# lzyhha/VisualCloze

Hardware: AMD Instinct MI355X
Metric: denoising-steps/sec (higher is better)
Workload: dtype bf16; 1 GPU; 384-grid-2x3 in-context, 30 solver points = 29 Flux evaluations per grid, L=512+3456 tokens, FLUX.1-Fill-dev geometry + LoRA r256 (merged), random-init weights, 1 independent grid(s) per GPU (data-parallel, no in-step collective); global_batch=1, seq_len=3968, parallelism=dp1

## Files before the change

visualcloze_amd/csrc/api.hip:

```cpp
#include "vcloze_internal.h"
#include <string.h>

static thread_local char g_err[512] = "";
#define ERRBUF g_err, (int)sizeof(g_err)
static inline hipStream_t S(void* s) { return (hipStream_t)s; }
static int hip_fail(const char* what, hipError_t e) {
  snprintf(g_err, sizeof(g_err), "%s: %s", what, hipGetErrorString(e));
  return VC_ERR_HIP;
}

extern "C" {

int vc_abi_version(void) { return VC_ABI_VERSION; }
const char* vc_last_error(void) { return g_err; }
void vc_struct_sizes(int32_t out[7]) {
  out[0] = (int32_t)sizeof(VcGemmProblem); out[1] = (int32_t)sizeof(VcGemmArgs); out[2] = (int32_t)sizeof(VcLnStream);
  out[3] = (int32_t)sizeof(VcAttention); out[4] = (int32_t)sizeof(VcFluxConfig); out[5] = (int32_t)sizeof(VcFluxInputs);
  out[6] = (int32_t)sizeof(VcFluxLaunchClass);
}

int vc_device_count(void) {
  int n = 0;
  hipError_t e = hipGetDeviceCount(&n);
  if (e != hipSuccess) { hip_fail("hipGetDeviceCount", e); return 0; }
  return n;
}
int vc_device_info(int dev, char* name, int namelen, int* cu_count, int64_t* hbm_bytes) {
  hipDeviceProp_t p;
  hipError_t e = hipGetDeviceProperties(&p, dev);
  if (e != hipSuccess) return hip_fail("hipGetDeviceProperties", e);
  if (name && namelen > 0) { strncpy(name, p.gcnArchName, namelen - 1); name[namelen - 1] = 0; }
  if (cu_count) *cu_count = p.multiProcessorCount;
  if (hbm_bytes) *hbm_bytes = (int64_t)p.totalGlobalMem;
  return VC_OK;
}

int vc_gemm(const VcGemmArgs* args, int tile_cfg, void* stream) {
  if (!args) { snprintf(g_err, sizeof(g_err), "gemm: null args"); return VC_ERR_ARG; }
  return vc_gemm_launch(*args, tile_cfg, S(stream), ERRBUF);
}
int vc_gemm_plan(const VcGemmArgs* args, int tile_cfg, int32_t out[8]) {
  if (!args || !out) { snprintf(g_err, sizeof(g_err), "gemm_plan: null argument"); return VC_ERR_ARG; }
  return vc_gemm_plan_impl(*args, tile_cfg, out, ERRBUF);
}
int vc_ln_modulate(const void* x, int64_t ldx, void* y, int64_t ldy, const void* shift, const void* scale,
                   int64_t mod_bstride, int32_t rows, int32_t D, int32_t rows_per_batch, const int32_t* step_ptr,
                   int64_t mod_step_stride, void* stream) {
  return vc_ln_modulate_launch(x, ldx, y, ldy, shift, scale, mod_bstride, rows, D, rows_per_batch, step_ptr,
                               mod_step_stride, S(stream), ERRBUF);
}
int vc_ln_modulate2(const VcLnStream* a, const VcLnStream* b, int64_t mod_bstride, int32_t D, const int32_t* step_ptr,
                    int64_t mod_step_stride, void* stream) {
  return vc_ln_modulate2_launch(a, b, mod_bstride, D, step_ptr, mod_step_stride, S(stream), ERRBUF);
}
int vc_qknorm_rope_vt(void* qkv, int64_t ld, int64_t bstride, const void* q_scale, const void* k_scale,
                      const void* q_scale2, const void* k_scale2, int32_t split, const float* rope,
                      int64_t rope_bstride, void* vt, int32_t B, int32_t L, int32_t Lpad, int32_t H, int32_t parts, void* stream) {
  return vc_qknorm_rope_vt_launch(qkv, ld, bstride, q_scale, k_scale, q_scale2, k_scale2, split, rope, rope_bstride, vt, B, L, Lpad, H,
                                  parts, S(stream), ERRBUF);
}
int vc_attention(const VcAttention* a, void* stream) {
  if (!a) { snprintf(g_err, sizeof(g_err), "attention: null args"); return VC_ERR_ARG; }
  return vc_attention_launch(*a, S(stream), ERRBUF);
}
int64_t vc_attention_scratch_bytes(void) { return vc_attention_scratch_bytes_impl(); }
int vc_timestep_embedding(const float* t, const float* freqs, void* out_bf16, int32_t n, int32_t half,
                          int32_t round_t_bf16, void* stream) {
  return vc_temb_launch(t, freqs, out_bf16, n, half, round_t_bf16, S(stream), ERRBUF);
}
int vc_silu(const void* x, void* y, int64_t n, void* stream) { return vc_silu_launch(x, y, n, S(stream), ERRBUF); }
int vc_act2d(const void* x, int64_t ldx, void* y, int64_t ldy, int32_t rows, int32_t cols, int32_t act, void* stream) {
  return vc_act2d_launch(x, ldx, y, ldy, rows, cols, act, S(stream), ERRBUF);
}
int vc_gate_residual(const void* y, int64_t ldy, const void* res, int64_t ldres, const void* gate, void* out, int64_t ldo,
                     int32_t rows, int32_t cols, const int32_t* step_ptr, int64_t gate_step_stride, void* stream) {
  return vc_gate_residual_launch(y, ldy, res, ldres, gate, out, ldo, rows, cols, step_ptr, gate_step_stride, S(stream), ERRBUF);
}
int vc_add3(const void* a, const void* b, const void* c, void* y, int64_t n, int64_t bn, int64_t cn, void* stream) {
  return vc_add3_launch(a, b, c, y, n, bn, cn, S(stream), ERRBUF);
}
int vc_copy(void* dst, const void* src, int64_t bytes, void* stream) {
  if (!dst || !src || bytes <= 0) { snprintf(g_err, sizeof(g_err), "copy: bad args"); return VC_ERR_ARG; }
  hipError_t e = hipMemcpyAsync(dst, src, (size_t)bytes, hipMemcpyDeviceToDevice, S(stream));
  return e == hipSuccess ? VC_OK : hip_fail("hipMemcpyAsync", e);
}
int vc_concat_cols(const void* x, int32_t cx, const void* cond, int32_t cc, void* out, int64_t rows, void* stream) {
  return vc_concat_cols_launch(x, cx, cond, cc, out, rows, S(stream), ERRBUF);
}
int vc_euler_step(void* x, const void* v, const float* dts, const int32_t* step_ptr, int64_t n, void* stream) {
  return vc_euler_launch(x, v, dts, step_ptr, n, S(stream), ERRBUF);
}
int vc_euler_step_f32(float* x32, void* shadow, const void* v, const float* dts, const int32_t* step_ptr, int64_t n, void* stream) {
  return vc_euler_f32_launch(x32, shadow, v, dts, step_ptr, n, S(stream), ERRBUF);
}
int vc_solver_evals(int method) {
  if (vc_evals_of(method)) return vc_evals_of(method);
  snprintf(g_err, sizeof(g_err), "solver_evals: unknown method %d (VC_SOLVER_EULER, VC_SOLVER_MIDPOINT, VC_SOLVER_RK4)", method);
  return VC_ERR_ARG;
}
int vc_ode_stage(int32_t method, int32_t stage, void* y, int32_t state_is_bf16, const void* v, void* k, void* y_in,
                 const float* dts, const int32_t* eval_ptr, int64_t n, void* stream) {
  return vc_ode_stage_launch(method, stage, y, state_is_bf16, v, k, y_in, dts, eval_ptr, n, S(stream), ERRBUF);
}
int vc_step_advance(int32_t* step_ptr, void* stream) { return vc_step_advance_launch(step_ptr, S(stream), ERRBUF); }
int vc_residual_change(const void* h0, const void* h1, const void* p, void* r, float* sums, float* metric, float* scratch, int32_t B,
                       int64_t n, void* stream) {
  return vc_residual_change_launch(h0, h1, p, r, sums, metric, scratch, B, n, S(stream), ERRBUF);
}
int vc_residual_sub(const void* a, int64_t a_bstride, const void* b, int64_t b_bstride, void* out, int64_t out_bstride, int32_t B,
                    int64_t n, void* stream) {
  return vc_residual_op_launch(0, a, a_bstride, b, b_bstride, out, out_bstride, B, n, S(stream), ERRBUF);
}
int vc_residual_add(const void* a, int64_t a_bstride, const void* b, int64_t b_bstride, void* out, int64_t out_bstride, int32_t B,
                    int64_t n, void* stream) {
  return vc_residual_op_launch(1, a, a_bstride, b, b_bstride, out, out_bstride, B, n, S(stream), ERRBUF);
}

int vc_sdedit_mix(const void* noise, const void* latent, float strength, void* out, int64_t n, void* stream) {
  return vc_sdedit_mix_launch(noise, latent, strength, out, n, S(stream), ERRBUF);
}
int vc_im2col3x3(const void* src, void* dst, int32_t H, int32_t W, int32_t C, int32_t up, void* stream) {
  return vc_im2col3x3_launch(src, dst, H, W, C, up, S(stream), ERRBUF);
}
int vc_groupnorm(const void* x, const void* gamma, const void* beta, void* y, void* scratch, int64_t scratch_bytes,
                 int64_t HW, int32_t C, int32_t G, float eps, int32_t swish, void* stream) {
  return vc_groupnorm_launch(x, gamma, beta, y, scratch, scratch_bytes, HW, C, G, eps, swish, S(stream), ERRBUF);
}
int vc_softmax_rows(void* x, int64_t ld, int32_t rows, int32_t cols, float scale, const void* bias, int64_t ld_bias,
                    int32_t causal_period, void* stream) {
  return vc_softmax_rows_launch(x, ld, rows, cols, scale, bias, ld_bias, causal_period, S(stream), ERRBUF);
}
int vc_embedding(const int32_t* ids, const void* table, int64_t ld_table, int32_t vocab, void* out, int32_t L, int32_t D, void* stream) {
  return vc_embedding_launch(ids, table, ld_table, vocab, out, L, D, S(stream), ERRBUF);
}
int vc_rmsnorm(const void* x, const void* weight, void* y, int32_t rows, int32_t D, float eps, void* stream) {
  return vc_rownorm_launch(x, weight, nullptr, y, rows, D, eps, 0, S(stream), ERRBUF);
}
int vc_layernorm(const void* x, const void* weight, const void* bias, void* y, int32_t rows, int32_t D, float eps, void* stream) {
  return vc_rownorm_launch(x, weight, bias, y, rows, D, eps, 1, S(stream), ERRBUF);
}
int vc_mul(const void* a, const void* b, void* y, int64_t n, void* stream) { return vc_ewise_launch(a, b, y, n, 0, S(stream), ERRBUF); }
int vc_add(const void* a, const void* b, void* y, int64_t n, void* stream) { return vc_ewise_launch(a, b, y, n, 1, S(stream), ERRBUF); }
int vc_quick_gelu(const void* x, void* y, int64_t n, void* stream) { return vc_ewise_launch(x, nullptr, y, n, 2, S(stream), ERRBUF); }
int vc_transpose(const void* src, int64_t ld_src, void* dst, int64_t ld_dst, int32_t rows, int32_t cols, void* stream) {
  return vc_transpose_launch(src, ld_src, dst, ld_dst, rows, cols, S(stream), ERRBUF);
}
int vc_nchw_to_nhwc(const void* src, int32_t src_is_f32, void* dst, int32_t C, int32_t Cp, int64_t HW, float div, float add, void* stream) {
  return vc_nchw_to_nhwc_launch(src, src_is_f32, dst, C, Cp, HW, div, add, S(stream), ERRBUF);
}
int vc_nhwc_to_nchw(const void* src, void* dst, int32_t dst_is_f32, int32_t C, int32_t Cp, int64_t HW, void* stream) {
  return vc_nhwc_to_nchw_launch(src, dst, dst_is_f32, C, Cp, HW, S(stream), ERRBUF);
}
int vc_gaussian_sample(const void* moments, int32_t Cp, const void* noise, void* out, int32_t Z, int64_t HW, float scale, float shift, void* stream) {
  return vc_gaussian_sample_launch(moments, Cp, noise, out, Z, HW, scale, shift, S(stream), ERRBUF);
}
int vc_conv3x3(const void* x, const void* w, const void* bias, void* out, int64_t ldc, const void* res, int64_t ldres,
               const void* gate, int32_t H, int32_t W, int32_t C, int32_t O, int32_t mode, void* stream) {
  return vc_conv3x3_launch(x, w, bias, out, ldc, res, ldres, gate, H, W, C, O, mode, S(stream), ERRBUF);
}
int vc_pack_latent(const void* latent, void* tokens, int32_t C, int32_t h, int32_t w, int64_t ld, int32_t col0, void* stream) {
  return vc_pack_latent_launch(latent, tokens, C, h, w, ld, col0, S(stream), ERRBUF);
}
int vc_pack_mask(const void* mask, void* tokens, int32_t H, int32_t W, int64_t ld, int32_t col0, void* stream) {
  return vc_pack_mask_launch(mask, tokens, H, W, ld, col0, S(stream), ERRBUF);
}
int vc_unpack_latent(const void* tokens, int64_t ld, int32_t col0, void* latent, int32_t C, int32_t h, int32_t w, void* stream) {
  return vc_unpack_latent_launch(tokens, ld, col0, latent, C, h, w, S(stream), ERRBUF);
}
int vc_lora_merge(const void* w, int32_t w_is_f32, int64_t ldw, const void* lora_a, int64_t lda, const void* lora_b, int64_t ldb,
                  float scale, void* out, int64_t ldo, const void* bias, int32_t bias_is_f32, const void* lora_b_bias, void* bias_out,
                  int32_t out_features, int32_t in_features, int32_t rank, void* stream) {
  return vc_lora_merge_launch(w, w_is_f32, ldw, lora_a, lda, lora_b, ldb, scale, out, ldo, bias, bias_is_f32, lora_b_bias, bias_out,
                              out_features, in_features, rank, S(stream), ERRBUF);
}

int vc_flux_create(const VcFluxConfig* cfg, void** handle) { return vc_flux_create_impl(cfg, handle, ERRBUF); }
int vc_flux_destroy(void* handle) { return vc_flux_destroy_impl(handle, ERRBUF); }
int vc_flux_bind_weight(void* handle, const char* name, const void* w, const void* bias, int32_t rows, int32_t cols, int64_t ldw) {
  return vc_flux_bind_weight_impl(handle, name, w, bias, rows, cols, ldw, ERRBUF);
}
int64_t vc_flux_mod_offset(void* handle, const char* module_name) { return vc_flux_mod_offset_impl(handle, module_name); }
int vc_flux_set_option(void* handle, const char* name, int32_t value) { return vc_flux_set_option_impl(handle, name, value, ERRBUF); }
int64_t vc_flux_workspace_bytes(void* handle, int32_t B, int32_t T, int32_t N, int32_t max_steps) {
  return vc_flux_workspace_bytes_impl(handle, B, T, N, max_steps);
}
int vc_flux_prepare(void* handle, const VcFluxInputs* in, void* workspace, int64_t workspace_bytes, void* stream) {
  return vc_flux_prepare_impl(handle, in, workspace, workspace_bytes, S(stream), ERRBUF);
}
int vc_flux_forward(void* handle, const void* img, const float* timesteps, int32_t timesteps_is_bf16, void* out, void* stream) {
  return vc_flux_forward_impl(handle, img, timesteps, timesteps_is_bf16, out, S(stream), ERRBUF);
}
int vc_flux_sample_begin(void* handle, const void* x, const void* cond, const float* t_grid, int32_t n_points, int32_t state_is_bf16,
                         void* stream) {
  return vc_flux_sample_begin_impl(handle, VC_SOLVER_EULER, x, cond, t_grid, n_points, state_is_bf16, S(stream), ERRBUF);
}
int vc_flux_sample_begin_ode(void* handle, int32_t method, const void* x, const void* cond, const float* t_grid, int32_t n_points,
                             int32_t state_is_bf16, void* stream) {
  return vc_flux_sample_begin_impl(handle, method, x, cond, t_grid, n_points, state_is_bf16, S(stream), ERRBUF);
}
int vc_flux_sample_steps(void* handle, int32_t n_steps, void* trajectory, void* stream) {
  return vc_flux_sample_steps_impl(handle, n_steps, trajectory, S(stream), ERRBUF);
}
int vc_flux_profile(void* handle, int32_t evaluations, VcFluxLaunchClass* out, int32_t capacity, int32_t* count, void* stream) {
  return vc_flux_profile_impl(handle, evaluations, out, capacity, count, S(stream), ERRBUF);
}
int vc_flux_sample_end(void* handle, void* x_out, void* stream) { return vc_flux_sample_end_impl(handle, x_out, S(stream), ERRBUF); }
int vc_flux_set_step_cache(void* handle, float threshold, int32_t max_consecutive) {
  return vc_flux_set_step_cache_impl(handle, threshold, max_consecutive, ERRBUF);
}
int vc_flux_step_cache_stats(void* handle, int32_t* computed, int32_t* reused, float* metrics, int32_t capacity) {
  return vc_flux_step_cache_stats_impl(handle, computed, reused, metrics, capacity, ERRBUF);
}
int vc_flux_sample_ode(void* handle, int32_t method, void* x, const void* cond, const float* t_grid, int32_t n_points,
                       int32_t state_is_bf16, void* trajectory, void* stream) {
  int rc = vc_flux_sample_begin_impl(handle, method, x, cond, t_grid, n_points, state_is_bf16, S(stream), ERRBUF);
  if (rc == VC_OK) rc = vc_flux_sample_steps_impl(handle, n_points - 1, trajectory, S(stream), ERRBUF);
  if (rc == VC_OK) rc = vc_flux_sample_end_impl(handle, x, S(stream), ERRBUF);
  return rc;
}
int vc_flux_sample_euler(void* handle, void* x, const void* cond, const float* t_grid, int32_t n_points, int32_t state_is_bf16,
                         void* trajectory, void* stream) {
  return vc_flux_sample_ode(handle, VC_SOLVER_EULER, x, cond, t_grid, n_points, state_is_bf16, trajectory, stream);
}

int vc_stream_create(void** stream) {
  if (!stream) { snprintf(g_err, sizeof(g_err), "stream_create: null"); return VC_ERR_ARG; }
  hipStream_t s;
  hipError_t e = hipStreamCreateWithFlags(&s, hipStreamNonBlocking);
  if (e != hipSuccess) return hip_fail("hipStreamCreate", e);
  *stream = (void*)s;
  return VC_OK;
}
int vc_stream_destroy(void* stream) {
  hipError_t e = hipStreamDestroy(S(stream));
  return e == hipSuccess ? VC_OK : hip_fail("hipStreamDestroy", e);
}
int vc_stream_sync(void* stream) {
  hipError_t e = hipStreamSynchronize(S(stream));
  return e == hipSuccess ? VC_OK : hip_fail("hipStreamSynchronize", e);
}
int vc_graph_begin(void* stream) {
  hipError_t e = hipStreamBeginCapture(S(stream), hipStreamCaptureModeThreadLocal);
  return e == hipSuccess ? VC_OK : hip_fail("hipStreamBeginCapture", e);
}
int vc_graph_end(void* stream, void** graph_exec) {
  if (!graph_exec) { snprintf(g_err, sizeof(g_err), "graph_end: null"); return VC_ERR_ARG; }
  hipGraph_t g = nullptr;
  hipError_t e = hipStreamEndCapture(S(stream), &g);
  if (e != hipSuccess) return hip_fail("hipStreamEndCapture", e);
  hipGraphExec_t ge = nullptr;
  e = hipGraphInstantiate(&ge, g, nullptr, nullptr, 0);
  (void)hipGraphDestroy(g);
  if (e != hipSuccess) return hip_fail("hipGraphInstantiate", e);
  *graph_exec = (void*)ge;
  return VC_OK;
}
int vc_graph_launch(void* graph_exec, void* stream) {
  hipError_t e = hipGraphLaunch((hipGraphExec_t)graph_exec, S(stream));
  return e == hipSuccess ? VC_OK : hip_fail("hipGraphLaunch", e);
}
int vc_graph_destroy(void* graph_exec) {
  hipError_t e = hipGraphExecDestroy((hipGraphExec_t)graph_exec);
  return e == hipSuccess ? VC_OK : hip_fail("hipGraphExecDestroy", e);
}
int vc_event_create(void** ev) {
  if (!ev) { snprintf(g_err, sizeof(g_err), "event_create: null"); return VC_ERR_ARG; }
  hipEvent_t e_;
  hipError_t e = hipEventCreate(&e_);
  if (e != hipSuccess) return hip_fail("hipEventCreate", e);
  *ev = (void*)e_;
  return VC_OK;
}
int vc_event_record(void* ev, void* stream) {
  hipError_t e = hipEventRecord((hipEvent_t)ev, S(stream));
  return e == hipSuccess ? VC_OK : hip_fail("hipEventRecord", e);
}
int vc_event_elapsed_ms(void* ev_start, void* ev_stop, float* ms) {
  hipError_t e = hipEventSynchronize((hipEvent_t)ev_stop);
  if (e != hipSuccess) return hip_fail("hipEventSynchronize", e);
  e = hipEventElapsedTime(ms, (hipEvent_t)ev_start, (hipEvent_t)ev_stop);
  return e == hipSuccess ? VC_OK : hip_fail("hipEventElapsedTime", e);
}
int vc_event_destroy(void* ev) {
  hipError_t e = hipEventDestroy((hipEvent_t)ev);
  return e == hipSuccess ? VC_OK : hip_fail("hipEventDestroy", e);
}

}
```

visualcloze_amd/csrc/flux_engine.hip:

```cpp
#include "common.h"
#include "vcloze_internal.h"
#include <math.h>
#include <string.h>
#include <string>
#include <unordered_map>
#include <vector>

namespace {

struct Lin {
  const void* w = nullptr;
  const void* b = nullptr;
  int N = 0, K = 0;
  int64_t ldw = 0;
};

struct DoubleW { Lin qkv[2], proj[2], mlp0[2], mlp2[2]; const void* qs[2]; const void* ks[2]; int64_t mod[2]; float bound; };
struct SingleW { Lin qkv, mlp, lin2; const void* qs; const void* ks; int64_t mod; float bound; };

struct Err {
  char* buf; int len;
};

struct Buffers {
  bf16_t *XI, *XT, *X, *XH, *QKV, *VT, *CAT, *HID, *TXT0, *XIN, *V, *XS, *COND, *MOD, *TEMB, *H1, *TVEC, *GVEC, *YVEC, *VEC, *GE, *GH, *YH, *KS, *YIN;
  float *ROPE, *TS, *DTS, *G32, *FREQS, *XS32;
  int32_t *STEP, *KVLEN, *KVGAP;
  bf16_t *SC_P = nullptr, *SC_R = nullptr, *SC_RS = nullptr;
  float *SC_PART = nullptr, *SC_METRIC = nullptr;
  void* ATT_SCRATCH = nullptr;
  int64_t att_scratch_bytes = 0;
  void* SK_WS = nullptr;
  int64_t sk_ws_bytes = 0;
};

struct Flux : Buffers {
  VcFluxConfig cfg{};
  int D = 0, H = 0, mlp = 0;
  int64_t n_mod = 0;
  std::unordered_map<std::string, Lin> bound;
  std::unordered_map<std::string, int64_t> mod_off;
  bool resolved = false;
  Lin img_in, txt_in, time_in[2], vector_in[2], guidance_in[2], final_lin, modulation;
  std::vector<DoubleW> dbl;
  std::vector<SingleW> sgl;
  int64_t final_mod = 0;
  int attn_variant = -1, tile_cfg = 0, fuse_qnorm = 2, fuse_vt = 1, qkv_heads = 0, fuse_knorm = 0, logit_bound_milli = 0, mlp_first = 0, splitk = 1, n_cu = 256;
  bool prepared = false;
  bool ws_sized = false;
  int B = 0, T = 0, N = 0, L = 0, Lp = 0, S = 0;
  bool ragged = false, gapped = false;
  char* base = nullptr;
  hipGraphExec_t graph = nullptr;
  struct Step { hipGraphExec_t g[3] = {nullptr, nullptr, nullptr}; } step;
  struct Key {
    char* base; int B, T, N, S, ragged, gapped, variant, tile, fuse, fuse_vt, state_f32, qkv_heads, fuse_knorm, bound, mlp_first, splitk, method, cache; hipStream_t s;
    bool operator==(const Key& o) const {
      return base == o.base && B == o.B && T == o.T && N == o.N && S == o.S && ragged == o.ragged && gapped == o.gapped &&
             variant == o.variant && tile == o.tile && fuse == o.fuse && fuse_vt == o.fuse_vt && state_f32 == o.state_f32 &&
             qkv_heads == o.qkv_heads && fuse_knorm == o.fuse_knorm && bound == o.bound && mlp_first == o.mlp_first && splitk == o.splitk && method == o.method && cache == o.cache && s == o.s;
    }
  } key{};
  std::vector<std::pair<Key, Step>> graphs;
  int steps_total = 0, steps_done = 0;
  bool state_f32 = false;
  int method = VC_SOLVER_EULER, evals = 1;
  float sc_threshold = 0.0f; int sc_max = 0;
  bool sc_on() const { return sc_threshold > 0.0f && sc_max != 0; }
  bool ws_cache = false;
  bool sc_active = false, sc_have = false;
  float sc_thr = 0.0f; int sc_lim = 0, sc_run = 0;
  int sc_computed = 0, sc_reused = 0;
  std::vector<float> sc_metrics;
  float* sc_host = nullptr;
  char* pinned = nullptr;
  size_t pinned_bytes = 0, pinned_used = 0;
  hipEvent_t staged = nullptr;
  bool staged_pending = false;
  struct ProfRec { int kind, epi, n, k; double flops, bytes; size_t e0; };
  bool prof_on = false;
  std::vector<hipEvent_t> prof_ev;
  size_t prof_used = 0;
  std::vector<ProfRec> prof_recs;
};

#define FAIL(code, ...)                         \
  do {                                          \
    snprintf(e.buf, e.len, __VA_ARGS__);        \
    return code;                                \
  } while (0)
#define TRY(x)                \
  do {                        \
    int rc_ = (x);            \
    if (rc_ != VC_OK) return rc_; \
  } while (0)
#define HIP(x, what)                                                        \
  do {                                                                      \
    hipError_t he_ = (x);                                                   \
    if (he_ != hipSuccess) FAIL(VC_ERR_HIP, what ": %s", hipGetErrorString(he_)); \
  } while (0)

inline int64_t align256(int64_t v) { return (v + 255) & ~(int64_t)255; }

struct Carver {
  char* base; int64_t off = 0;
  template <class T> T* take(int64_t count) {
    T* p = base ? (T*)(base + off) : nullptr;
    off += align256(count * (int64_t)sizeof(T));
    return p;
  }
};

int64_t carve(Buffers& f, const Flux& g, char* base, int B, int T, int N, int S) {
  const int64_t D = g.D, H = g.H, mlp = g.mlp, L = T + N, Lp = (L + 63) / 64 * 64;
  const int64_t in_ch = g.cfg.in_channels, out_ch = g.cfg.out_channels;
  Carver c{base};
  f.XI = c.take<bf16_t>(B * N * D);          f.XT = c.take<bf16_t>(B * T * D);
  f.X = c.take<bf16_t>(B * L * D);           f.XH = c.take<bf16_t>(B * L * D);
  f.QKV = c.take<bf16_t>(B * L * 3 * D);     f.VT = c.take<bf16_t>(B * H * 128 * Lp);
  f.CAT = c.take<bf16_t>(B * L * (D + mlp)); f.HID = c.take<bf16_t>(B * L * mlp);
  f.TXT0 = c.take<bf16_t>(B * T * D);        f.XIN = c.take<bf16_t>(B * N * in_ch);
  f.V = c.take<bf16_t>(B * N * out_ch);      f.XS = c.take<bf16_t>(B * N * out_ch);
  f.COND = c.take<bf16_t>(B * N * (in_ch - out_ch));
  f.MOD = c.take<bf16_t>((int64_t)S * B * g.n_mod);
  f.TEMB = c.take<bf16_t>((int64_t)S * B * 256);
  f.H1 = c.take<bf16_t>((int64_t)S * B * D); f.TVEC = c.take<bf16_t>((int64_t)S * B * D);
  f.VEC = c.take<bf16_t>((int64_t)S * B * D);
  f.GVEC = c.take<bf16_t>(B * D);            f.YVEC = c.take<bf16_t>(B * D);
  f.GE = c.take<bf16_t>(B * 256);            f.GH = c.take<bf16_t>(B * D);  f.YH = c.take<bf16_t>(B * D);
  f.ROPE = c.take<float>(B * L * 128);
  f.TS = c.take<float>((int64_t)S * B);      f.DTS = c.take<float>(S);
  f.G32 = c.take<float>(B);                  f.FREQS = c.take<float>(128);
  f.XS32 = c.take<float>(B * N * out_ch);
  f.KS = c.take<bf16_t>(3 * B * N * out_ch); f.YIN = c.take<bf16_t>(B * N * out_ch);
  f.STEP = c.take<int32_t>(1);               f.KVLEN = c.take<int32_t>(B);  f.KVGAP = c.take<int32_t>(2 * B);
  f.att_scratch_bytes = vc_attention_scratch_bytes_impl();
  f.ATT_SCRATCH = c.take<char>(f.att_scratch_bytes);
  auto sk = g.bound.find("splitk_ws");
  if (sk != g.bound.end()) { f.SK_WS = const_cast<void*>(sk->second.w); f.sk_ws_bytes = (int64_t)sk->second.N * sk->second.K * 4; }
  else { f.SK_WS = c.take<char>(VC_GEMM_SPLITK_WS_BYTES); f.sk_ws_bytes = VC_GEMM_SPLITK_WS_BYTES; }
  if (g.sc_on()) {
    f.SC_P = c.take<bf16_t>(B * N * D); f.SC_R = c.take<bf16_t>(B * N * D); f.SC_RS = c.take<bf16_t>(B * N * D);
    f.SC_PART = c.take<float>((int64_t)B * 2 * VC_RESIDUAL_CHANGE_MAX_BLOCKS); f.SC_METRIC = c.take<float>(1);
  }
  return c.off;
}

int find(Flux& f, const std::string& name, Lin& out, int N, int K, bool need_bias, Err e) {
  auto it = f.bound.find(name);
  if (it == f.bound.end()) FAIL(VC_ERR_STATE, "flux: weight '%s' is not bound", name.c_str());
  out = it->second;
  if (out.N != N || out.K != K) FAIL(VC_ERR_ARG, "flux: weight '%s' is [%d, %d], expected [%d, %d]", name.c_str(), out.N, out.K, N, K);
  if (need_bias && !out.b) FAIL(VC_ERR_ARG, "flux: weight '%s' needs a bias", name.c_str());
  return VC_OK;
}
int find_scale(Flux& f, const std::string& name, const void*& out, Err e) {
  auto it = f.bound.find(name);
  if (it == f.bound.end()) FAIL(VC_ERR_STATE, "flux: scale '%s' is not bound", name.c_str());
  if (it->second.N * it->second.K != 128) FAIL(VC_ERR_ARG, "flux: scale '%s' must hold 128 values", name.c_str());
  out = it->second.w;
  return VC_OK;
}

void layout_modulation(Flux& f) {
  int64_t o = 0;
  for (int i = 0; i < f.cfg.depth; ++i) {
    f.mod_off["double_blocks." + std::to_string(i) + ".img_mod.lin"] = o; o += 6 * f.D;
    f.mod_off["double_blocks." + std::to_string(i) + ".txt_mod.lin"] = o; o += 6 * f.D;
  }
  for (int i = 0; i < f.cfg.depth_single_blocks; ++i) { f.mod_off["single_blocks." + std::to_string(i) + ".modulation.lin"] = o; o += 3 * f.D; }
  f.mod_off["final_layer.adaLN_modulation.1"] = o; o += 2 * f.D;
  f.n_mod = o;
}

int scale_absmax(const void* dev, double& out, Err e) {
  uint16_t h[128];
  HIP(hipMemcpy(h, dev, sizeof(h), hipMemcpyDeviceToHost), "hipMemcpy (QK-norm scale)");
  out = 0;
  bool nan = false;
  for (int i = 0; i < 128; ++i) {
    uint32_t u = (uint32_t)h[i] << 16;
    float v;
    memcpy(&v, &u, 4);
    const double a = v < 0 ? -(double)v : (double)v;
    if (a != a) nan = true;
    else if (a > out) out = a;
  }
  if (nan) out = 1e30;
  return VC_OK;
}
inline float logit_bound_of(double qmax, double kmax) { return (float)(1.02 * 11.313708498984761 * 1.4426950408889634 * qmax * kmax); }

int resolve(Flux& f, Err e) {
  if (f.resolved) return VC_OK;
  const int D = f.D, mlp = f.mlp;
  TRY(find(f, "img_in", f.img_in, D, f.cfg.in_channels, false, e));
  TRY(find(f, "txt_in", f.txt_in, D, f.cfg.context_in_dim, false, e));
  TRY(find(f, "time_in.in_layer", f.time_in[0], D, 256, false, e));
  TRY(find(f, "time_in.out_layer", f.time_in[1], D, D, false, e));
  TRY(find(f, "vector_in.in_layer", f.vector_in[0], D, f.cfg.vec_in_dim, false, e));
  TRY(find(f, "vector_in.out_layer", f.vector_in[1], D, D, false, e));
  if (f.cfg.guidance_embed) {
    TRY(find(f, "guidance_in.in_layer", f.guidance_in[0], D, 256, false, e));
    TRY(find(f, "guidance_in.out_layer", f.guidance_in[1], D, D, false, e));
  }
  TRY(find(f, "final_layer.linear", f.final_lin, f.cfg.out_channels, D, false, e));
  TRY(find(f, "modulation", f.modulation, (int)f.n_mod, D, false, e));
  f.dbl.assign(f.cfg.depth, DoubleW{});
  for (int i = 0; i < f.cfg.depth; ++i) {
    const std::string pf = "double_blocks." + std::to_string(i) + ".";
    const char* st[2] = {"img", "txt"};
    for (int k = 0; k < 2; ++k) {
      const std::string a = pf + st[k] + "_attn.", m = pf + st[k] + "_mlp.";
      TRY(find(f, a + "qkv", f.dbl[i].qkv[k], 3 * D, D, false, e));
      TRY(find(f, a + "proj", f.dbl[i].proj[k], D, D, false, e));
      TRY(find(f, m + "0", f.dbl[i].mlp0[k], mlp, D, false, e));
      TRY(find(f, m + "2", f.dbl[i].mlp2[k], D, mlp, false, e));
      TRY(find_scale(f, a + "norm.query_norm.scale", f.dbl[i].qs[k], e));
      TRY(find_scale(f, a + "norm.key_norm.scale", f.dbl[i].ks[k], e));
      f.dbl[i].mod[k] = f.mod_off[pf + st[k] + "_mod.lin"];
    }
    double q[2], k2[2];
    for (int k = 0; k < 2; ++k) { TRY(scale_absmax(f.dbl[i].qs[k], q[k], e)); TRY(scale_absmax(f.dbl[i].ks[k], k2[k], e)); }
    f.dbl[i].bound = logit_bound_of(q[0] > q[1] ? q[0] : q[1], k2[0] > k2[1] ? k2[0] : k2[1]);
  }
  f.sgl.assign(f.cfg.depth_single_blocks, SingleW{});
  for (int i = 0; i < f.cfg.depth_single_blocks; ++i) {
    const std::string pf = "single_blocks." + std::to_string(i) + ".";
    Lin l1;
    TRY(find(f, pf + "linear1", l1, 3 * D + mlp, D, false, e));
    SingleW& w = f.sgl[i];
    w.qkv = l1; w.qkv.N = 3 * D;
    w.mlp = l1; w.mlp.N = mlp;
    w.mlp.w = (const bf16_t*)l1.w + (int64_t)3 * D * l1.ldw;
    w.mlp.b = l1.b ? (const void*)((const bf16_t*)l1.b + 3 * D) : nullptr;
    TRY(find(f, pf + "linear2", w.lin2, D, D + mlp, false, e));
    TRY(find_scale(f, pf + "norm.query_norm.scale", w.qs, e));
    TRY(find_scale(f, pf + "norm.key_norm.scale", w.ks, e));
    w.mod = f.mod_off[pf + "modulation.lin"];
    double q, k;
    TRY(scale_absmax(w.qs, q, e)); TRY(scale_absmax(w.ks, k, e));
    w.bound = logit_bound_of(q, k);
  }
  f.final_mod = f.mod_off["final_layer.adaLN_modulation.1"];
  f.resolved = true;
  return VC_OK;
}

int attention_variant(const Flux& f);
bool kn_in_gemm(const Flux& f) { return f.fuse_knorm && f.qkv_heads > 0 && (attention_variant(f) & 8); }
bool qn_in_gemm(const Flux& f) { return kn_in_gemm(f) && f.fuse_qnorm >= 2; }
int qkv_epi(const Flux& f) { return f.fuse_vt || f.qkv_heads > 0 ? VC_EPI_QKV : VC_EPI_BIAS; }
void with_vt(Flux& f, VcGemmProblem& p, int rows, int row0, const void* q_scale, const void* k_scale) {
  if (f.fuse_vt) { p.vt = f.VT; p.vt_bstride = (int64_t)f.H * 128 * f.Lp; p.vt_col0 = 2 * f.D; p.vt_lpad = f.Lp; }
  if (f.qkv_heads > 0) {
    p.kn_heads = f.qkv_heads;
    if (kn_in_gemm(f)) { p.kn_scale = k_scale; p.kn_rope = f.ROPE; p.kn_rope_bstride = (int64_t)f.L * 128; }
    if (qn_in_gemm(f)) { p.qn_scale = q_scale; p.qn_prescale = 1; }
  }
  if (f.fuse_vt || f.qkv_heads > 0) { p.vt_rpb = rows; p.vt_row0 = row0; }
}

VcGemmProblem prob(const void* A, int64_t lda, const Lin& w, void* C, int64_t ldc, int M) {
  VcGemmProblem p;
  memset(&p, 0, sizeof(p));
  p.A = A; p.W = w.w; p.bias = w.b; p.C = C;
  p.lda = lda; p.ldw = w.ldw; p.ldc = ldc;
  p.M = M; p.N = w.N; p.K = w.K;
  p.rows_per_batch = M;
  return p;
}
int prof_event(Flux& f, hipStream_t s, Err e) {
  if (f.prof_used == f.prof_ev.size()) {
    hipEvent_t ev;
    HIP(hipEventCreate(&ev), "hipEventCreate");
    f.prof_ev.push_back(ev);
  }
  HIP(hipEventRecord(f.prof_ev[f.prof_used++], s), "hipEventRecord");
  return VC_OK;
}
int prof_open(Flux& f, hipStream_t s, int kind, int epi, int n, int k, double flops, double bytes, Err e) {
  if (!f.prof_on) return VC_OK;
  f.prof_recs.push_back(Flux::ProfRec{kind, epi, n, k, flops, bytes, f.prof_used});
  return prof_event(f, s, e);
}
int prof_close(Flux& f, hipStream_t s, Err e) { return f.prof_on ? prof_event(f, s, e) : VC_OK; }

int gemm(Flux& f, const VcGemmProblem* ps, int n, int epi, const int32_t* step_ptr, int64_t gate_step_stride, hipStream_t s, Err e) {
  VcGemmArgs a;
  memset(&a, 0, sizeof(a));
  for (int i = 0; i < n; ++i) a.p[i] = ps[i];
  a.nprob = n; a.epi = epi; a.step_ptr = step_ptr; a.gate_step_stride = gate_step_stride;
  if (f.splitk) { a.splitk_ws = f.SK_WS; a.splitk_ws_bytes = f.sk_ws_bytes; }
  double flops = 0;
  for (int i = 0; i < n; ++i) flops += 2.0 * ps[i].M * ps[i].N * ps[i].K;
  TRY(prof_open(f, s, VC_LAUNCH_GEMM, epi, ps[0].N, ps[0].K, flops, 0, e));
  TRY(vc_gemm_launch(a, f.tile_cfg, s, e.buf, e.len));
  return prof_close(f, s, e);
}
int lin(Flux& f, const Lin& w, const void* A, int64_t lda, void* C, int64_t ldc, int M, int epi, hipStream_t s, Err e) {
  VcGemmProblem p = prob(A, lda, w, C, ldc, M);
  return gemm(f, &p, 1, epi, nullptr, 0, s, e);
}

struct Ctx {
  const int32_t* step_ptr;
  hipStream_t s;
  int64_t mss;
};
inline const bf16_t* modp(Flux& f, int64_t off, int idx) { return f.MOD + off + (int64_t)idx * f.D; }

int ln2(Flux& f, const Ctx& c, const DoubleW& w, int idx, Err e) {
  VcLnStream a{f.XI, f.D, f.XH, f.D, modp(f, w.mod[0], idx), modp(f, w.mod[0], idx + 1), f.B * f.N, f.N};
  VcLnStream b{f.XT, f.D, f.XH + (int64_t)f.B * f.N * f.D, f.D, modp(f, w.mod[1], idx), modp(f, w.mod[1], idx + 1), f.B * f.T, f.T};
  TRY(prof_open(f, c.s, VC_LAUNCH_LN_MODULATE, 0, 0, 0, 0, 4.0 * f.B * f.L * f.D, e));
  TRY(vc_ln_modulate2_launch(&a, &b, f.n_mod, f.D, c.step_ptr, c.mss, c.s, e.buf, e.len));
  return prof_close(f, c.s, e);
}
int ln1(Flux& f, const Ctx& c, int64_t mod, Err e) {
  TRY(prof_open(f, c.s, VC_LAUNCH_LN_MODULATE, 0, 0, 0, 0, 4.0 * f.B * f.L * f.D, e));
  TRY(vc_ln_modulate_launch(f.X, f.D, f.XH, f.D, modp(f, mod, 0), modp(f, mod, 1), f.n_mod, f.B * f.L, f.D, f.L, c.step_ptr, c.mss,
                            c.s, e.buf, e.len));
  return prof_close(f, c.s, e);
}

int attention_variant(const Flux& f) {
  if (f.attn_variant >= 0) return f.attn_variant;
  const int items = ((f.L + 255) / 256) * f.H * f.B;
  return items >= f.n_cu ? 28 : 2 * items >= f.n_cu ? 8 : 3;
}

int attention(Flux& f, const Ctx& c, const void* q1, const void* k1, const void* q2, const void* k2, int split, float block_bound, Err e) {
  const int variant = attention_variant(f);
  const bool fused_q = (variant & 8) && f.fuse_qnorm, q_done = qn_in_gemm(f);
  const int64_t ld = 3 * f.D, ldo = f.D + f.mlp;
  const int parts = (kn_in_gemm(f) ? 0 : VC_QKN_K) | (fused_q ? 0 : VC_QKN_Q) | (f.fuse_vt ? 0 : VC_QKN_VT);
  if (parts)
    TRY(vc_qknorm_rope_vt_launch(f.QKV, ld, f.L * ld, q1, k1, q2, k2, split, f.ROPE, (int64_t)f.L * 128, f.VT, f.B, f.L, f.Lp, f.H,
                                 parts, c.s, e.buf, e.len));
  VcAttention a;
  memset(&a, 0, sizeof(a));
  a.qkv = f.QKV; a.ld = ld; a.bstride = f.L * ld;
  a.vt = f.VT; a.out = f.CAT; a.ldo = ldo; a.out_bstride = f.L * ldo;
  a.kv_len = f.ragged ? f.KVLEN : nullptr;
  a.kv_gap = f.gapped ? f.KVGAP : nullptr;
  a.B = f.B; a.L = f.L; a.Lpad = f.Lp; a.H = f.H; a.variant = variant;
  a.scratch = f.ATT_SCRATCH; a.scratch_bytes = f.att_scratch_bytes;
  if (q_done) a.q_prescaled = 1;
  else if (fused_q) { a.q_scale = q1; a.q_scale2 = q2; a.split = split; a.rope = f.ROPE; a.rope_bstride = (int64_t)f.L * 128; }
  const float cap = (float)f.logit_bound_milli * 1e-3f;
  a.logit_bound = f.logit_bound_milli > 0 ? (block_bound < cap ? block_bound : cap) : 0.0f;
  if (f.logit_bound_milli > 0 && !(block_bound < 1e30f)) a.logit_bound = 1e30f;
  TRY(prof_open(f, c.s, VC_LAUNCH_ATTENTION, variant, 0, 0, 4.0 * f.L * f.L * f.D * f.B, 0, e));
  TRY(vc_attention_launch(a, c.s, e.buf, e.len));
  return prof_close(f, c.s, e);
}

int double_block(Flux& f, const Ctx& c, const DoubleW& w, Err e) {
  const int B = f.B, T = f.T, N = f.N, L = f.L, D = f.D, mlp = f.mlp;
  const int64_t ldq = 3 * D, ldc = D + mlp;
  bf16_t* XH_I = f.XH; bf16_t* XH_T = f.XH + (int64_t)B * N * D;
  bf16_t* HID_I = f.HID; bf16_t* HID_T = f.HID + (int64_t)B * N * mlp;
  bf16_t* streams[2] = {f.XI, f.XT};
  const int rows[2] = {N, T};
  TRY(ln2(f, c, w, 0, e));
  {
    VcGemmProblem p[2] = {prob(XH_I, D, w.qkv[0], f.QKV + (int64_t)T * ldq, ldq, B * N), prob(XH_T, D, w.qkv[1], f.QKV, ldq, B * T)};
    p[0].c_rpb = N; p[1].c_rpb = T;
    p[0].c_bstride = p[1].c_bstride = (int64_t)L * ldq;
    with_vt(f, p[0], N, T, w.qs[0], w.ks[0]); with_vt(f, p[1], T, 0, w.qs[1], w.ks[1]);
    TRY(gemm(f, p, 2, qkv_epi(f), nullptr, 0, c.s, e));
  }
  TRY(attention(f, c, w.qs[1], w.ks[1], w.qs[0], w.ks[0], T, w.bound, e));
  {
    VcGemmProblem p[2] = {prob(f.CAT + (int64_t)T * ldc, ldc, w.proj[0], f.XI, D, B * N), prob(f.CAT, ldc, w.proj[1], f.XT, D, B * T)};
    for (int k = 0; k < 2; ++k) {
      p[k].res = streams[k]; p[k].ldres = D; p[k].gate = modp(f, w.mod[k], 2); p[k].gate_bstride = f.n_mod;
      p[k].rows_per_batch = rows[k]; p[k].a_rpb = rows[k]; p[k].a_bstride = (int64_t)L * ldc;
    }
    TRY(gemm(f, p, 2, VC_EPI_GATE_RES, c.step_ptr, c.mss, c.s, e));
  }
  TRY(ln2(f, c, w, 3, e));
  {
    VcGemmProblem p[2] = {prob(XH_I, D, w.mlp0[0], HID_I, mlp, B * N), prob(XH_T, D, w.mlp0[1], HID_T, mlp, B * T)};
    TRY(gemm(f, p, 2, VC_EPI_GELU, nullptr, 0, c.s, e));
  }
  {
    VcGemmProblem p[2] = {prob(HID_I, mlp, w.mlp2[0], f.XI, D, B * N), prob(HID_T, mlp, w.mlp2[1], f.XT, D, B * T)};
    for (int k = 0; k < 2; ++k) {
      p[k].res = streams[k]; p[k].ldres = D; p[k].gate = modp(f, w.mod[k], 5); p[k].gate_bstride = f.n_mod; p[k].rows_per_batch = rows[k];
    }
    TRY(gemm(f, p, 2, VC_EPI_GATE_RES, c.step_ptr, c.mss, c.s, e));
  }
  return VC_OK;
}

int single_block(Flux& f, const Ctx& c, const SingleW& w, Err e) {
  const int M = f.B * f.L, D = f.D, mlp = f.mlp;
  const int64_t ldc = D + mlp;
  TRY(ln1(f, c, w.mod, e));
  {
    VcGemmProblem p = prob(f.XH, D, w.qkv, f.QKV, 3 * D, M);
    with_vt(f, p, f.L, 0, w.qs, w.ks);
    TRY(gemm(f, &p, 1, qkv_epi(f), nullptr, 0, c.s, e));
  }
  if (f.mlp_first) TRY(lin(f, w.mlp, f.XH, D, f.CAT + D, ldc, M, VC_EPI_GELU, c.s, e));
  TRY(attention(f, c, w.qs, w.ks, nullptr, nullptr, 0, w.bound, e));
  if (!f.mlp_first) TRY(lin(f, w.mlp, f.XH, D, f.CAT + D, ldc, M, VC_EPI_GELU, c.s, e));
  VcGemmProblem p = prob(f.CAT, ldc, w.lin2, f.X, D, M);
  p.res = f.X; p.ldres = D; p.gate = modp(f, w.mod, 2); p.gate_bstride = f.n_mod; p.rows_per_batch = f.L;
  return gemm(f, &p, 1, VC_EPI_GATE_RES, c.step_ptr, c.mss, c.s, e);
}

int d2d(void* dst, const void* src, int64_t bytes, hipStream_t s, Err e) {
  HIP(hipMemcpyAsync(dst, src, (size_t)bytes, hipMemcpyDeviceToDevice, s), "hipMemcpyAsync");
  return VC_OK;
}

int eval_inputs(Flux& f, bool concat, const void* img_rows, hipStream_t s, Err e) {
  const int B = f.B, T = f.T, N = f.N, D = f.D;
  const int in_ch = f.cfg.in_channels, out_ch = f.cfg.out_channels;
  if (concat) TRY(vc_concat_cols_launch(f.method == VC_SOLVER_EULER ? f.XS : f.YIN, out_ch, f.COND, in_ch - out_ch, f.XIN, (int64_t)B * N, s, e.buf, e.len));
  TRY(d2d(f.XT, f.TXT0, (int64_t)B * T * D * 2, s, e));
  return lin(f, f.img_in, img_rows ? img_rows : f.XIN, in_ch, f.XI, D, B * N, VC_EPI_BIAS, s, e);
}
int eval_blocks(Flux& f, const Ctx& c, size_t first, Err e) {
  const int B = f.B, T = f.T, N = f.N, L = f.L, D = f.D;
  hipStream_t s = c.s;
  for (size_t i = first; i < f.dbl.size(); ++i) TRY(double_block(f, c, f.dbl[i], e));
  for (int b = 0; b < B; ++b) {
    TRY(d2d(f.X + (int64_t)b * L * D, f.XT + (int64_t)b * T * D, (int64_t)T * D * 2, s, e));
    TRY(d2d(f.X + ((int64_t)b * L + T) * D, f.XI + (int64_t)b * N * D, (int64_t)N * D * 2, s, e));
  }
  for (auto& w : f.sgl) TRY(single_block(f, c, w, e));
  return VC_OK;
}
int eval_output(Flux& f, const Ctx& c, void* out, bool euler, Err e) {
  const int B = f.B, T = f.T, N = f.N, L = f.L, D = f.D;
  const int out_ch = f.cfg.out_channels;
  const int32_t* step_ptr = c.step_ptr;
  hipStream_t s = c.s;
  TRY(ln1(f, c, f.final_mod, e));
  VcGemmProblem p = prob(f.XH + (int64_t)T * D, D, f.final_lin, out ? out : f.V, out_ch, B * N);
  p.a_rpb = N; p.a_bstride = (int64_t)L * D;
  TRY(gemm(f, &p, 1, VC_EPI_BIAS, nullptr, 0, s, e));
  if (euler && f.method != VC_SOLVER_EULER) {
    TRY(vc_ode_stage_launch(f.method, -1, f.state_f32 ? (void*)f.XS32 : (void*)f.XS, !f.state_f32, f.V, f.KS, f.YIN, f.DTS, step_ptr,
                            (int64_t)B * N * out_ch, s, e.buf, e.len));
    TRY(vc_step_advance_launch((int32_t*)step_ptr, s, e.buf, e.len));
  } else if (euler) {
    if (f.state_f32) TRY(vc_euler_f32_launch(f.XS32, f.XS, f.V, f.DTS, step_ptr, (int64_t)B * N * out_ch, s, e.buf, e.len));
    else TRY(vc_euler_launch(f.XS, f.V, f.DTS, step_ptr, (int64_t)B * N * out_ch, s, e.buf, e.len));
    TRY(vc_step_advance_launch((int32_t*)step_ptr, s, e.buf, e.len));
  }
  return VC_OK;
}
int evaluate(Flux& f, const int32_t* step_ptr, bool concat, const void* img_rows, void* out, bool euler, hipStream_t s, Err e) {
  Ctx c{step_ptr, s, (int64_t)f.B * f.n_mod};
  TRY(eval_inputs(f, concat, img_rows, s, e));
  TRY(eval_blocks(f, c, 0, e));
  return eval_output(f, c, out, euler, e);
}

int cache_head(Flux& f, hipStream_t s, Err e) {
  const int64_t nd = (int64_t)f.N * f.D;
  Ctx c{f.STEP, s, (int64_t)f.B * f.n_mod};
  TRY(eval_inputs(f, true, nullptr, s, e));
  TRY(d2d(f.X, f.XI, f.B * nd * 2, s, e));
  TRY(double_block(f, c, f.dbl[0], e));
  TRY(vc_residual_change_launch(f.X, f.XI, f.SC_P, f.SC_RS, nullptr, f.SC_METRIC, f.SC_PART, f.B, nd, s, e.buf, e.len));
  HIP(hipMemcpyAsync(f.sc_host, f.SC_METRIC, sizeof(float), hipMemcpyDeviceToHost, s), "hipMemcpyAsync(D2H)");
  return VC_OK;
}
int cache_tail_compute(Flux& f, bool euler, hipStream_t s, Err e) {
  const int64_t nd = (int64_t)f.N * f.D;
  Ctx c{f.STEP, s, (int64_t)f.B * f.n_mod};
  TRY(d2d(f.SC_P, f.SC_RS, f.B * nd * 2, s, e));
  TRY(d2d(f.SC_RS, f.XI, f.B * nd * 2, s, e));
  TRY(eval_blocks(f, c, 1, e));
  TRY(vc_residual_op_launch(0, f.X + (int64_t)f.T * f.D, (int64_t)f.L * f.D, f.SC_RS, nd, f.SC_R, nd, f.B, nd, s, e.buf, e.len));
  return eval_output(f, c, nullptr, euler, e);
}
int cache_tail_reuse(Flux& f, bool euler, hipStream_t s, Err e) {
  const int64_t nd = (int64_t)f.N * f.D;
  Ctx c{f.STEP, s, (int64_t)f.B * f.n_mod};
  TRY(vc_residual_op_launch(1, f.XI, nd, f.SC_R, nd, f.X + (int64_t)f.T * f.D, (int64_t)f.L * f.D, f.B, nd, s, e.buf, e.len));
  return eval_output(f, c, nullptr, euler, e);
}

int stage_begin(Flux& f, size_t bytes, Err e) {
  if (f.staged_pending) { HIP(hipEventSynchronize(f.staged), "hipEventSynchronize"); f.staged_pending = false; }
  if (bytes > f.pinned_bytes) {
    if (f.pinned) (void)hipHostFree(f.pinned);
    f.pinned = nullptr; f.pinned_bytes = 0;
    HIP(hipHostMalloc((void**)&f.pinned, bytes, hipHostMallocDefault), "hipHostMalloc");
    f.pinned_bytes = bytes;
  }
  f.pinned_used = 0;
  return VC_OK;
}
template <class T> T* stage_take(Flux& f, size_t count) {
  T* p = (T*)(f.pinned + f.pinned_used);
  f.pinned_used += (size_t)align256((int64_t)(count * sizeof(T)));
  return p;
}
int stage_send(Flux& f, void* dst, const void* staged, size_t bytes, hipStream_t s, Err e) {
  HIP(hipMemcpyAsync(dst, staged, bytes, hipMemcpyHostToDevice, s), "hipMemcpyAsync(H2D)");
  return VC_OK;
}
int stage_end(Flux& f, hipStream_t s, Err e) {
  HIP(hipEventRecord(f.staged, s), "hipEventRecord");
  f.staged_pending = true;
  return VC_OK;
}

inline float bf16_round(float v) {
  uint32_t u;
  memcpy(&u, &v, 4);
  u += 0x7fffu + ((u >> 16) & 1u);
  u &= 0xffff0000u;
  memcpy(&v, &u, 4);
  return v;
}

int time_precompute(Flux& f, int S, int timesteps_is_bf16, hipStream_t s, Err e) {
  const int B = f.B, D = f.D, M = S * B;
  TRY(vc_temb_launch(f.TS, f.FREQS, f.TEMB, M, 128, timesteps_is_bf16, s, e.buf, e.len));
  TRY(lin(f, f.time_in[0], f.TEMB, 256, f.H1, D, M, VC_EPI_SILU, s, e));
  TRY(lin(f, f.time_in[1], f.H1, D, f.TVEC, D, M, VC_EPI_BIAS, s, e));
  if (f.cfg.guidance_embed)
    TRY(vc_add3_launch(f.TVEC, f.GVEC, f.YVEC, f.VEC, (int64_t)M * D, (int64_t)B * D, (int64_t)B * D, s, e.buf, e.len));
  else
    TRY(vc_add3_launch(f.TVEC, f.YVEC, nullptr, f.VEC, (int64_t)M * D, (int64_t)B * D, 1, s, e.buf, e.len));
  TRY(vc_silu_launch(f.VEC, f.H1, (int64_t)M * D, s, e.buf, e.len));
  return lin(f, f.modulation, f.H1, D, f.MOD, f.n_mod, M, VC_EPI_BIAS, s, e);
}

constexpr size_t MAX_GRAPHS = 4;
void drop_prof(Flux& f) {
  for (auto ev : f.prof_ev) (void)hipEventDestroy(ev);
  f.prof_ev.clear();
}
void drop_graph(Flux& f) {
  for (auto& g : f.graphs)
    for (auto ge : g.second.g) if (ge) (void)hipGraphExecDestroy(ge);
  f.graphs.clear();
  f.graph = nullptr;
  f.step = Flux::Step{};
}

template <class F> int capture(hipStream_t s, hipGraphExec_t& out, Err e, F issue) {
  HIP(hipStreamBeginCapture(s, hipStreamCaptureModeThreadLocal), "hipStreamBeginCapture");
  const int rc = issue();
  hipGraph_t g = nullptr;
  hipError_t he = hipStreamEndCapture(s, &g);
  if (rc != VC_OK) { if (g) (void)hipGraphDestroy(g); return rc; }
  HIP(he, "hipStreamEndCapture");
  he = hipGraphInstantiate(&out, g, nullptr, nullptr, 0);
  (void)hipGraphDestroy(g);
  HIP(he, "hipGraphInstantiate");
  return VC_OK;
}
int step_graph(Flux& f, hipStream_t s, Err e) {
  Flux::Key k{f.base, f.B, f.T, f.N, f.S, f.ragged, f.gapped, attention_variant(f), f.tile_cfg, f.fuse_qnorm, f.fuse_vt, f.state_f32,
              f.qkv_heads, f.fuse_knorm, f.logit_bound_milli, f.mlp_first, f.splitk, f.method, f.sc_active, s};
  for (size_t i = 0; i < f.graphs.size(); ++i)
    if (f.graphs[i].first == k) {
      auto hit = f.graphs[i];
      f.graphs.erase(f.graphs.begin() + i);
      f.graphs.insert(f.graphs.begin(), hit);
      f.step = hit.second; f.graph = f.step.g[0]; f.key = k;
      return VC_OK;
    }
  f.graph = nullptr;
  f.step = Flux::Step{};
  Flux::Step st;
  int rc = VC_OK;
  if (!f.sc_active) {
    TRY(evaluate(f, f.STEP, true, nullptr, nullptr, false, s, e));
    rc = capture(s, st.g[0], e, [&] { return evaluate(f, f.STEP, true, nullptr, nullptr, true, s, e); });
  } else {
    TRY(cache_head(f, s, e));
    TRY(cache_tail_compute(f, false, s, e));
    TRY(cache_tail_reuse(f, false, s, e));
    rc = capture(s, st.g[0], e, [&] { return cache_head(f, s, e); });
    if (rc == VC_OK) rc = capture(s, st.g[1], e, [&] { return cache_tail_compute(f, true, s, e); });
    if (rc == VC_OK) rc = capture(s, st.g[2], e, [&] { return cache_tail_reuse(f, true, s, e); });
  }
  if (rc != VC_OK) {
    for (auto ge : st.g) if (ge) (void)hipGraphExecDestroy(ge);
    return rc;
  }
  if (f.graphs.size() >= MAX_GRAPHS) {
    for (auto ge : f.graphs.back().second.g) if (ge) (void)hipGraphExecDestroy(ge);
    f.graphs.pop_back();
  }
  f.graphs.insert(f.graphs.begin(), {k, st});
  f.step = st; f.graph = st.g[0]; f.key = k;
  return VC_OK;
}

}

#define H(handle)                                                         \
  Err e{err, errlen};                                                     \
  if (!(handle)) FAIL(VC_ERR_ARG, "flux: null handle");                   \
  Flux& f = *(Flux*)(handle)

int vc_flux_create_impl(const VcFluxConfig* cfg, void** handle, char* err, int errlen) {
  Err e{err, errlen};
  if (!cfg || !handle) FAIL(VC_ERR_ARG, "flux_create: null argument");
  if (cfg->hidden_size <= 0 || cfg->num_heads <= 0 || cfg->hidden_size != cfg->num_heads * 128)
    FAIL(VC_ERR_ARG, "flux_create: hidden_size must be num_heads * 128 (the gfx950 attention kernels are specialised for head_dim 128)");
  if (cfg->axes_dim[0] + cfg->axes_dim[1] + cfg->axes_dim[2] != 128 || (cfg->axes_dim[0] | cfg->axes_dim[1] | cfg->axes_dim[2]) & 1)
    FAIL(VC_ERR_ARG, "flux_create: axes_dim must be even and sum to 128");
  if (cfg->in_channels <= cfg->out_channels || cfg->out_channels <= 0 || cfg->depth < 0 || cfg->depth_single_blocks < 0 || cfg->mlp_hidden <= 0)
    FAIL(VC_ERR_ARG, "flux_create: bad channel / depth configuration");
  Flux* f = new Flux();
  f->cfg = *cfg;
  f->D = cfg->hidden_size; f->H = cfg->num_heads; f->mlp = cfg->mlp_hidden;
  layout_modulation(*f);
  int dev = 0;
  hipDeviceProp_t p;
  if (hipGetDevice(&dev) != hipSuccess || hipGetDeviceProperties(&p, dev) != hipSuccess) {
    delete f;
    FAIL(VC_ERR_HIP, "flux_create: no ROCm device");
  }
  f->n_cu = p.multiProcessorCount;
  if (hipEventCreateWithFlags(&f->staged, hipEventDisableTiming) != hipSuccess) { delete f; FAIL(VC_ERR_HIP, "flux_create: hipEventCreate failed"); }
  *handle = f;
  return VC_OK;
}

int vc_flux_destroy_impl(void* handle, char* err, int errlen) {
  H(handle);
  if (f.staged_pending) (void)hipEventSynchronize(f.staged);
  drop_graph(f);
  drop_prof(f);
  if (f.pinned) (void)hipHostFree(f.pinned);
  if (f.sc_host) (void)hipHostFree(f.sc_host);
  if (f.staged) (void)hipEventDestroy(f.staged);
  delete &f;
  return VC_OK;
}

int vc_flux_bind_weight_impl(void* handle, const char* name, const void* w, const void* bias, int32_t rows, int32_t cols, int64_t ldw,
                             char* err, int errlen) {
  H(handle);
  if (!name || !w || rows <= 0 || cols <= 0 || ldw < cols) FAIL(VC_ERR_ARG, "flux_bind_weight: bad arguments for '%s'", name ? name : "?");
  if (!strcmp(name, "splitk_ws") && f.ws_sized && f.bound.find("splitk_ws") == f.bound.end())
    FAIL(VC_ERR_STATE, "flux_bind_weight: bind 'splitk_ws' BEFORE the first vc_flux_workspace_bytes / vc_flux_prepare (it changes the size and "
                       "layout of every workspace)");
  Lin l;
  l.w = w; l.b = bias; l.N = rows; l.K = cols; l.ldw = ldw;
  f.bound[name] = l;
  f.resolved = false;
  f.prepared = false;
  drop_graph(f);
  return VC_OK;
}

int64_t vc_flux_mod_offset_impl(void* handle, const char* name) {
  if (!handle) return -1;
  Flux& f = *(Flux*)handle;
  if (!name) return f.n_mod;
  auto it = f.mod_off.find(name);
  return it == f.mod_off.end() ? -1 : it->second;
}

int vc_flux_set_option_impl(void* handle, const char* name, int32_t value, char* err, int errlen) {
  H(handle);
  if (!name) FAIL(VC_ERR_ARG, "flux_set_option: null name");
  if (!strcmp(name, "attn_variant")) f.attn_variant = value;
  else if (!strcmp(name, "tile_cfg")) f.tile_cfg = value;
  else if (!strcmp(name, "fuse_qnorm")) f.fuse_qnorm = value < 0 ? 0 : value > 2 ? 2 : value;
  else if (!strcmp(name, "fuse_vt")) f.fuse_vt = value != 0;
  else if (!strcmp(name, "qkv_heads")) {
    if (value != 0 && value != f.H) FAIL(VC_ERR_ARG, "flux_set_option: qkv_heads must be 0 or num_heads = %d", f.H);
    f.qkv_heads = value;
  } else if (!strcmp(name, "fuse_knorm")) f.fuse_knorm = value != 0;
  else if (!strcmp(name, "logit_bound_milli")) f.logit_bound_milli = value > 0 ? value : 0;
  else if (!strcmp(name, "mlp_first")) f.mlp_first = value != 0;
  else if (!strcmp(name, "splitk")) f.splitk = value != 0;
  else FAIL(VC_ERR_ARG, "flux_set_option: unknown option '%s'", name);
  return VC_OK;
}

int64_t vc_flux_workspace_bytes_impl(void* handle, int32_t B, int32_t T, int32_t N, int32_t max_steps) {
  if (!handle || B <= 0 || T <= 0 || N <= 0 || max_steps <= 0) return -1;
  Buffers tmp;
  ((Flux*)handle)->ws_sized = true;
  return carve(tmp, *(Flux*)handle, nullptr, B, T, N, max_steps);
}

int vc_flux_prepare_impl(void* handle, const VcFluxInputs* in, void* workspace, int64_t workspace_bytes, hipStream_t s, char* err, int errlen) {
  H(handle);
  if (!in || !workspace) FAIL(VC_ERR_ARG, "flux_prepare: null argument");
  f.ws_sized = true;
  const int B = in->B, T = in->T, N = in->N, S = in->max_steps;
  if (B <= 0 || T <= 0 || N <= 0 || S <= 0) FAIL(VC_ERR_ARG, "flux_prepare: B, T, N, max_steps must be positive");
  if (!in->txt || !in->y || !in->img_ids || !in->txt_ids) FAIL(VC_ERR_ARG, "flux_prepare: txt, y, img_ids, txt_ids are required");
  if (f.cfg.guidance_embed && !in->guidance) FAIL(VC_ERR_ARG, "Didn't get guidance strength for guidance distilled model.");
  if (in->kv_gap && !in->kv_len) FAIL(VC_ERR_ARG, "flux_prepare: kv_gap needs kv_len");
  if ((uintptr_t)workspace & 255) FAIL(VC_ERR_ARG, "flux_prepare: workspace must be 256-byte aligned");
  TRY(resolve(f, e));
  f.prepared = false;
  const int64_t need = carve(f, f, (char*)workspace, B, T, N, S);
  if (workspace_bytes < need) FAIL(VC_ERR_ARG, "flux_prepare: workspace of %lld bytes, %lld needed", (long long)workspace_bytes, (long long)need);
  f.base = (char*)workspace;
  f.ws_cache = f.sc_on();
  f.B = B; f.T = T; f.N = N; f.L = T + N; f.Lp = (f.L + 63) / 64 * 64; f.S = S;
  const int L = f.L, D = f.D;
  f.ragged = f.gapped = false;
  for (int b = 0; b < B; ++b) {
    const int kv = in->kv_len ? in->kv_len[b] : L;
    if (kv < 0 || kv > L) FAIL(VC_ERR_ARG, "flux_prepare: kv_len[%d] = %d outside [0, %d]", b, kv, L);
    if (kv < L) f.ragged = true;
    if (in->kv_gap) {
      const int lo = in->kv_gap[2 * b], hi = in->kv_gap[2 * b + 1];
      if (lo < 0 || lo > hi || hi > kv) FAIL(VC_ERR_ARG, "flux_prepare: kv_gap[%d] = (%d, %d) must lie inside [0, kv_len = %d)", b, lo, hi, kv);
      if (hi > lo) f.gapped = true;
    }
  }
  if (f.gapped) f.ragged = true;
  const size_t n_rope = (size_t)B * L * 128;
  TRY(stage_begin(f, (n_rope + 128 + 4 * B + 64) * sizeof(float) + 8 * 256, e));
  float* rope = stage_take<float>(f, n_rope);
  {
    int pair0 = 0;
    std::vector<float> table;
    std::vector<int> slot((size_t)B * L);
    for (int ax = 0; ax < 3; ++ax) {
      const int half = f.cfg.axes_dim[ax] / 2, d = f.cfg.axes_dim[ax];
      std::unordered_map<float, int> seen;
      std::vector<float> values;
      for (int b = 0; b < B; ++b)
        for (int r = 0; r < L; ++r) {
          const float id = r < T ? in->txt_ids[((size_t)b * T + r) * 3 + ax] : in->img_ids[((size_t)b * N + (r - T)) * 3 + ax];
          auto it = seen.find(id);
          if (it == seen.end()) { it = seen.emplace(id, (int)values.size()).first; values.push_back(id); }
          slot[(size_t)b * L + r] = it->second;
        }
      table.resize(values.size() * (size_t)half * 2);
      for (int j = 0; j < half; ++j) {
        const double omega = 1.0 / pow((double)f.cfg.theta, (double)(2 * j) / (double)d);
        for (size_t v = 0; v < values.size(); ++v) {
          const double ang = (double)values[v] * omega;
          table[(v * half + j) * 2] = (float)cos(ang);
          table[(v * half + j) * 2 + 1] = (float)sin(ang);
        }
      }
      for (size_t row = 0; row < (size_t)B * L; ++row)
        memcpy(rope + (row * 64 + pair0) * 2, table.data() + (size_t)slot[row] * half * 2, (size_t)half * 2 * sizeof(float));
      pair0 += half;
    }
  }
  float* freqs = stage_take<float>(f, 128);
  for (int k = 0; k < 128; ++k)
    freqs[k] = (float)exp((double)((float)(-log(10000.0)) * (float)k / 128.0f));
  int32_t* kvl = stage_take<int32_t>(f, B);
  int32_t* gap = stage_take<int32_t>(f, 2 * B);
  float* g32 = stage_take<float>(f, B);
  for (int b = 0; b < B; ++b) {
    kvl[b] = in->kv_len ? in->kv_len[b] : L;
    gap[2 * b] = in->kv_gap ? in->kv_gap[2 * b] : 0;
    gap[2 * b + 1] = in->kv_gap ? in->kv_gap[2 * b + 1] : 0;
    g32[b] = in->guidance ? in->guidance[b] : 0.0f;
  }
  TRY(stage_send(f, f.ROPE, rope, n_rope * sizeof(float), s, e));
  {
    auto it = f.bound.find("timestep_freqs");
    if (it != f.bound.end()) {
      if (it->second.N * it->second.K != 128) FAIL(VC_ERR_ARG, "flux_prepare: 'timestep_freqs' must hold 128 f32 values");
      TRY(d2d(f.FREQS, it->second.w, 128 * sizeof(float), s, e));
    } else {
      TRY(stage_send(f, f.FREQS, freqs, 128 * sizeof(float), s, e));
    }
  }
  TRY(stage_send(f, f.KVLEN, kvl, B * sizeof(int32_t), s, e));
  TRY(stage_send(f, f.KVGAP, gap, 2 * B * sizeof(int32_t), s, e));
  TRY(stage_send(f, f.G32, g32, B * sizeof(float), s, e));
  TRY(stage_end(f, s, e));
  HIP(hipMemsetAsync(f.VT, 0, (size_t)B * f.H * 128 * f.Lp * 2, s), "hipMemsetAsync");
  HIP(hipMemsetAsync((char*)f.ATT_SCRATCH + vc_attention_flags_offset_impl(), 0, (size_t)vc_attention64_flags_bytes_impl(f.n_cu), s), "hipMemsetAsync");
  TRY(lin(f, f.txt_in, in->txt, f.cfg.context_in_dim, f.TXT0, D, B * T, VC_EPI_BIAS, s, e));
  if (f.cfg.guidance_embed) {
    TRY(vc_temb_launch(f.G32, f.FREQS, f.GE, B, 128, in->guidance_is_bf16, s, e.buf, e.len));
    TRY(lin(f, f.guidance_in[0], f.GE, 256, f.GH, D, B, VC_EPI_SILU, s, e));
    TRY(lin(f, f.guidance_in[1], f.GH, D, f.GVEC, D, B, VC_EPI_BIAS, s, e));
  }
  TRY(lin(f, f.vector_in[0], in->y, f.cfg.vec_in_dim, f.YH, D, B, VC_EPI_SILU, s, e));
  TRY(lin(f, f.vector_in[1], f.YH, D, f.YVEC, D, B, VC_EPI_BIAS, s, e));
  f.prepared = true;
  f.steps_total = f.steps_done = 0;
  return VC_OK;
}

int vc_flux_forward_impl(void* handle, const void* img, const float* timesteps, int32_t timesteps_is_bf16, void* out, hipStream_t s,
                         char* err, int errlen) {
  H(handle);
  if (!f.prepared) FAIL(VC_ERR_STATE, "flux_forward: call vc_flux_prepare first");
  if (!img || !timesteps || !out) FAIL(VC_ERR_ARG, "flux_forward: null argument");
  TRY(stage_begin(f, f.B * sizeof(float) + 256, e));
  float* ts = stage_take<float>(f, f.B);
  for (int b = 0; b < f.B; ++b) ts[b] = timesteps[b];
  TRY(stage_send(f, f.TS, ts, f.B * sizeof(float), s, e));
  TRY(stage_end(f, s, e));
  TRY(time_precompute(f, 1, timesteps_is_bf16, s, e));
  f.steps_total = f.steps_done = 0;
  return evaluate(f, nullptr, false, img, out, false, s, e);
}

void stage_times(int method, float t0, float t1, float dt, float* out) {
#pragma clang fp contract(off)
  out[0] = t0;
  if (method == VC_SOLVER_MIDPOINT) {
    volatile float half_dt = 0.5f * dt;
    out[1] = t0 + half_dt;
  } else if (method == VC_SOLVER_RK4) {
    volatile float a = dt * (float)(1.0 / 3.0), b = dt * (float)(2.0 / 3.0);
    out[1] = t0 + a; out[2] = t0 + b; out[3] = t1;
  }
}

int vc_flux_sample_begin_impl(void* handle, int32_t method, const void* x, const void* cond, const float* t_grid, int32_t n_points,
                              int32_t state_is_bf16, hipStream_t s, char* err, int errlen) {
  H(handle);
  const int E = vc_evals_of(method);
  if (!E) FAIL(VC_ERR_ARG, "flux_sample: unknown solver method %d (VC_SOLVER_EULER, VC_SOLVER_MIDPOINT, VC_SOLVER_RK4)", method);
  if (!f.prepared) FAIL(VC_ERR_STATE, "flux_sample: call vc_flux_prepare first");
  if (!x || !cond || !t_grid) FAIL(VC_ERR_ARG, "flux_sample: null argument");
  const int S = n_points - 1, B = f.B;
  if (S < 1 || (int64_t)S * E > f.S)
    FAIL(VC_ERR_ARG, "flux_sample: %d steps of %d evaluation(s), the prepared workspace holds 1..%d evaluations", S, E, f.S);
  const bool cached = f.sc_on();
  if (cached && method != VC_SOLVER_EULER)
    FAIL(VC_ERR_ARG, "flux_sample: the step cache works with VC_SOLVER_EULER only (method %d): turn it off with vc_flux_set_step_cache(handle, 0, 0)", method);
  if (cached && f.dbl.empty()) FAIL(VC_ERR_ARG, "flux_sample: the step cache needs at least one double block");
  if (cached && !f.ws_cache)
    FAIL(VC_ERR_STATE, "flux_sample: the step cache was turned on after vc_flux_prepare: ask vc_flux_workspace_bytes and prepare again");
  if (cached && !f.sc_host) HIP(hipHostMalloc((void**)&f.sc_host, 256, hipHostMallocDefault), "hipHostMalloc");
  const int SE = S * E;
  TRY(stage_begin(f, ((size_t)SE * B + S) * sizeof(float) + 512, e));
  float* ts = stage_take<float>(f, (size_t)SE * B);
  float* dts = stage_take<float>(f, S);
  for (int i = 0; i < S; ++i) {
    dts[i] = t_grid[i + 1] - t_grid[i];
    float te[4];
    stage_times(method, t_grid[i], t_grid[i + 1], dts[i], te);
    for (int j = 0; j < E; ++j) {
      const float tm = 1.0f - (state_is_bf16 ? bf16_round(te[j]) : te[j]);
      for (int b = 0; b < B; ++b) ts[((size_t)i * E + j) * B + b] = tm;
    }
  }
  TRY(stage_send(f, f.TS, ts, (size_t)SE * B * sizeof(float), s, e));
  TRY(stage_send(f, f.DTS, dts, S * sizeof(float), s, e));
  TRY(stage_end(f, s, e));
  TRY(time_precompute(f, SE, 0, s, e));
  const int64_t n = (int64_t)B * f.N;
  f.state_f32 = !state_is_bf16;
  f.method = method; f.evals = E;
  if (f.state_f32) {
    TRY(d2d(f.XS32, x, n * f.cfg.out_channels * 4, s, e));
    TRY(vc_euler_f32_launch(f.XS32, f.XS, nullptr, nullptr, nullptr, n * f.cfg.out_channels, s, e.buf, e.len));
  } else {
    TRY(d2d(f.XS, x, n * f.cfg.out_channels * 2, s, e));
  }
  if (E > 1) TRY(d2d(f.YIN, f.XS, n * f.cfg.out_channels * 2, s, e));
  TRY(d2d(f.COND, cond, n * (f.cfg.in_channels - f.cfg.out_channels) * 2, s, e));
  HIP(hipMemsetAsync(f.STEP, 0, sizeof(int32_t), s), "hipMemsetAsync");
  f.sc_active = cached; f.sc_thr = f.sc_threshold; f.sc_lim = f.sc_max;
  f.sc_have = false; f.sc_run = f.sc_computed = f.sc_reused = 0;
  f.sc_metrics.clear();
  if (s) TRY(step_graph(f, s, e));
  if (cached) HIP(hipMemsetAsync(f.SC_P, 0, (size_t)n * f.D * 2, s), "hipMemsetAsync");
  f.steps_total = S; f.steps_done = 0;
  return VC_OK;
}

static int cached_step(Flux& f, hipStream_t s, Err e) {
  if (s) HIP(hipGraphLaunch(f.step.g[0], s), "hipGraphLaunch");
  else TRY(cache_head(f, s, e));
  HIP(hipStreamSynchronize(s), "hipStreamSynchronize");
  const float m = *(volatile float*)f.sc_host;
  const bool reuse = f.sc_have && m < f.sc_thr && (f.sc_lim < 0 || f.sc_run < f.sc_lim);
  f.sc_metrics.push_back(f.sc_have ? m : NAN);
  if (s) HIP(hipGraphLaunch(f.step.g[reuse ? 2 : 1], s), "hipGraphLaunch");
  else if (reuse) TRY(cache_tail_reuse(f, true, s, e));
  else TRY(cache_tail_compute(f, true, s, e));
  if (reuse) { ++f.sc_reused; ++f.sc_run; }
  else { ++f.sc_computed; f.sc_run = 0; f.sc_have = true; }
  return VC_OK;
}

int vc_flux_sample_steps_impl(void* handle, int32_t n_steps, void* trajectory, hipStream_t s, char* err, int errlen) {
  H(handle);
  if (!f.prepared || f.steps_total == 0) FAIL(VC_ERR_STATE, "flux_sample_steps: call vc_flux_sample_begin first");
  if (n_steps < 0 || f.steps_done + n_steps > f.steps_total)
    FAIL(VC_ERR_ARG, "flux_sample_steps: %d more steps after %d of %d", n_steps, f.steps_done, f.steps_total);
  if (s && (!f.graph || f.key.s != s)) FAIL(VC_ERR_STATE, "flux_sample_steps: the step was captured on another stream");
  const int64_t state_bytes = (int64_t)f.B * f.N * f.cfg.out_channels * (f.state_f32 ? 4 : 2);
  const void* state = f.state_f32 ? (const void*)f.XS32 : (const void*)f.XS;
  for (int i = 0; i < n_steps; ++i) {
    for (int j = 0; j < f.evals; ++j) {
      if (f.sc_active) { TRY(cached_step(f, s, e)); continue; }
      if (s) HIP(hipGraphLaunch(f.graph, s), "hipGraphLaunch");
      else TRY(evaluate(f, f.STEP, true, nullptr, nullptr, true, s, e));
      ++f.sc_computed;
    }
    if (trajectory) TRY(d2d((char*)trajectory + (int64_t)i * state_bytes, state, state_bytes, s, e));
    ++f.steps_done;
  }
  return VC_OK;
}

int vc_flux_sample_end_impl(void* handle, void* x_out, hipStream_t s, char* err, int errlen) {
  H(handle);
  if (!f.prepared || f.steps_total == 0) FAIL(VC_ERR_STATE, "flux_sample_end: no sample in flight");
  if (!x_out) FAIL(VC_ERR_ARG, "flux_sample_end: null output");
  if (f.state_f32) return d2d(x_out, f.XS32, (int64_t)f.B * f.N * f.cfg.out_channels * 4, s, e);
  return d2d(x_out, f.XS, (int64_t)f.B * f.N * f.cfg.out_channels * 2, s, e);
}

int vc_flux_set_step_cache_impl(void* handle, float threshold, int32_t max_consecutive, char* err, int errlen) {
  H(handle);
  if (threshold != threshold) FAIL(VC_ERR_ARG, "flux_set_step_cache: threshold is NaN");
  f.sc_threshold = threshold > 0.0f ? threshold : 0.0f;
  f.sc_max = max_consecutive;
  return VC_OK;
}

int vc_flux_step_cache_stats_impl(void* handle, int32_t* computed, int32_t* reused, float* metrics, int32_t capacity, char* err, int errlen) {
  H(handle);
  if (capacity < 0 || (capacity > 0 && !metrics)) FAIL(VC_ERR_ARG, "flux_step_cache_stats: bad arguments");
  if (computed) *computed = f.sc_computed;
  if (reused) *reused = f.sc_reused;
  const int done = f.sc_computed + f.sc_reused;
  for (int i = 0; i < capacity; ++i) metrics[i] = i < done && i < (int)f.sc_metrics.size() ? f.sc_metrics[i] : NAN;
  return VC_OK;
}

int vc_flux_profile_impl(void* handle, int32_t evaluations, VcFluxLaunchClass* out, int32_t capacity, int32_t* count, hipStream_t s,
                         char* err, int errlen) {
  H(handle);
  if (!f.prepared || f.steps_total == 0) FAIL(VC_ERR_STATE, "flux_profile: call vc_flux_sample_begin first");
  if (!out || !count || capacity <= 0 || evaluations <= 0) FAIL(VC_ERR_ARG, "flux_profile: bad argument");
  TRY(evaluate(f, f.STEP, true, nullptr, nullptr, false, s, e));
  f.prof_recs.clear();
  f.prof_used = 0;
  f.prof_on = true;
  int rc = VC_OK;
  for (int i = 0; i < evaluations && rc == VC_OK; ++i) rc = evaluate(f, f.STEP, true, nullptr, nullptr, false, s, e);
  f.prof_on = false;
  if (rc != VC_OK) return rc;
  HIP(hipStreamSynchronize(s), "hipStreamSynchronize");
  int n = 0;
  for (const auto& r : f.prof_recs) {
    float ms = 0.f;
    HIP(hipEventElapsedTime(&ms, f.prof_ev[r.e0], f.prof_ev[r.e0 + 1]), "hipEventElapsedTime");
    const float us = ms * 1e3f;
    int j = 0;
    while (j < n && !(out[j].kind == r.kind && out[j].epi == r.epi && out[j].n == r.n && out[j].k == r.k)) ++j;
    if (j == n) {
      if (n == capacity) FAIL(VC_ERR_ARG, "flux_profile: more than %d launch classes", capacity);
      memset(&out[n], 0, sizeof(out[n]));
      out[n].kind = r.kind; out[n].epi = r.epi; out[n].n = r.n; out[n].k = r.k;
      out[n].min_us = us; out[n].max_us = us;
      ++n;
    }
    out[j].launches += 1;
    out[j].flops += r.flops;
    out[j].bytes += r.bytes;
    out[j].total_us += us;
    if (us < out[j].min_us) out[j].min_us = us;
    if (us > out[j].max_us) out[j].max_us = us;
  }
  *count = n;
  return VC_OK;
}
```

visualcloze_amd/csrc/norm.hip:

```cpp
#include "common.h"
#include "vcloze_internal.h"

namespace {

struct LnStream2 {
  const bf16_t* x; long ldx; bf16_t* y; long ldy; const bf16_t* shift; const bf16_t* scale; int rows; int rows_per_batch;
};

template <int NCH>
__global__ __launch_bounds__(256) void ln_modulate_kernel(const bf16_t* __restrict__ x, long ldx, bf16_t* __restrict__ y,
                                                          long ldy, const bf16_t* __restrict__ shift,
                                                          const bf16_t* __restrict__ scale, long mod_bstride, int rows,
                                                          int D, int rows_per_batch, const int* __restrict__ step_ptr,
                                                          long mod_step_stride, const LnStream2 second) {
  const int lane = threadIdx.x & 63;
  int row = blockIdx.x * 4 + (threadIdx.x >> 6);
  if (row >= rows) {
    row -= rows;
    if (row >= second.rows) return;
    x = second.x; ldx = second.ldx; y = second.y; ldy = second.ldy; shift = second.shift; scale = second.scale;
    rows_per_batch = second.rows_per_batch;
  }
  long moff = (long)(row / rows_per_batch) * mod_bstride;
  if (step_ptr) moff += (long)(*step_ptr) * mod_step_stride;
  const bf16_t* xr = x + (long)row * ldx;
  float v[NCH][8];
  float sum = 0.f;
#pragma unroll
  for (int c = 0; c < NCH; ++c) {
    const int idx = c * 512 + lane * 8;
    if (idx < D) {
      const u32x4 w = *(const u32x4*)(xr + idx);
#pragma unroll
      for (int e = 0; e < 4; ++e) { v[c][2 * e] = lo_bf(w[e]); v[c][2 * e + 1] = hi_bf(w[e]); }
#pragma unroll
      for (int e = 0; e < 8; ++e) sum += v[c][e];
    } else {
#pragma unroll
      for (int e = 0; e < 8; ++e) v[c][e] = 0.f;
    }
  }
  const float mean = wave_sum(sum) / (float)D;
  float ss = 0.f;
#pragma unroll
  for (int c = 0; c < NCH; ++c) {
    const int idx = c * 512 + lane * 8;
    if (idx < D) {
#pragma unroll
      for (int e = 0; e < 8; ++e) { const float d = v[c][e] - mean; ss += d * d; }
    }
  }
  const float rstd = 1.0f / sqrtf(wave_sum(ss) / (float)D + 1e-6f);
  bf16_t* yr = y + (long)row * ldy;
#pragma unroll
  for (int c = 0; c < NCH; ++c) {
    const int idx = c * 512 + lane * 8;
    if (idx < D) {
      const u32x4 sc = *(const u32x4*)(scale + moff + idx);
      const u32x4 sh = *(const u32x4*)(shift + moff + idx);
      u32x4 o;
#pragma unroll
      for (int e = 0; e < 4; ++e) {
        const float a0 = rbf(1.0f + lo_bf(sc[e])), a1 = rbf(1.0f + hi_bf(sc[e]));
        const float r0 = a0 * ((v[c][2 * e] - mean) * rstd) + lo_bf(sh[e]);
        const float r1 = a1 * ((v[c][2 * e + 1] - mean) * rstd) + hi_bf(sh[e]);
        o[e] = pack2bf(r0, r1);
      }
      *(u32x4*)(yr + idx) = o;
    }
  }
}

__global__ __launch_bounds__(256) void qknorm_rope_vt_kernel(bf16_t* __restrict__ qkv, long ld, long bstride,
                                                             const bf16_t* __restrict__ q_scale,
                                                             const bf16_t* __restrict__ k_scale,
                                                             const bf16_t* __restrict__ q_scale2,
                                                             const bf16_t* __restrict__ k_scale2, int split,
                                                             const float* __restrict__ rope, long rope_bstride,
                                                             bf16_t* __restrict__ vt, int L, int Lpad, int H, int parts) {
  __shared__ uint32_t tl[128 * 33];
  const int tid = threadIdx.x;
  const int t0 = blockIdx.x * 64, h = blockIdx.y, b = blockIdx.z;
  bf16_t* base = qkv + (long)b * bstride + h * 128;
  const int sub = tid & 15;

  for (int p = (parts & 1) ? 0 : 4; p < ((parts & 2) ? 8 : 4); ++p) {
    const int rowid = p * 16 + (tid >> 4);
    const int which = rowid >> 6;
    const int tok = t0 + (rowid & 63);
    const bool ok = tok < L;
    bf16_t* ptr = base + (long)(ok ? tok : 0) * ld + which * (H * 128) + sub * 8;
    const u32x4 w = *(const u32x4*)ptr;
    const bf16_t* sc = (tok < split ? (which ? k_scale : q_scale) : (which ? k_scale2 : q_scale2)) + sub * 8;
    const u32x4 sw = *(const u32x4*)sc;
    float g[8];
#pragma unroll
    for (int e = 0; e < 4; ++e) { g[2 * e] = lo_bf(sw[e]); g[2 * e + 1] = hi_bf(sw[e]); }
    const float* rp = rope + (long)b * rope_bstride + (long)(ok ? tok : 0) * 128 + sub * 8;
    const f32x4 c0 = *(const f32x4*)rp;
    const f32x4 c1 = *(const f32x4*)(rp + 4);
    const float cs[8] = {c0[0], c0[1], c0[2], c0[3], c1[0], c1[1], c1[2], c1[3]};
    const u32x4 o = qknorm_rope8(w, g, cs, (which == 0 && (parts & 8)) ? VC_QK_PRESCALE : 1.0f);
    if (ok) *(u32x4*)ptr = o;
  }

  if (!(parts & 4)) return;
  const bf16_t* vbase = base + 2 * (H * 128);
#pragma unroll
  for (int i = 0; i < 2; ++i) {
    const int pc = i * 256 + tid;
    const int dch = pc & 15, tp = pc >> 4;
    const int ta = t0 + 2 * tp, tb = ta + 1;
    u32x4 wa = {0, 0, 0, 0}, wb = {0, 0, 0, 0};
    if (ta < L) wa = *(const u32x4*)(vbase + (long)ta * ld + dch * 8);
    if (tb < L) wb = *(const u32x4*)(vbase + (long)tb * ld + dch * 8);
#pragma unroll
    for (int e = 0; e < 4; ++e) {
      const uint32_t lo = (wa[e] & 0xffffu) | (wb[e] << 16);
      const uint32_t hi = (wa[e] >> 16) | (wb[e] & 0xffff0000u);
      tl[(dch * 8 + 2 * e) * 33 + tp] = lo;
      tl[(dch * 8 + 2 * e + 1) * 33 + tp] = hi;
    }
  }
  __syncthreads();
  bf16_t* vout = vt + ((long)(b * H + h) * 128) * Lpad + t0;
#pragma unroll
  for (int i = 0; i < 4; ++i) {
    const int c = i * 256 + tid;
    const int d = c >> 3, part = c & 7;
    u32x4 w;
#pragma unroll
    for (int e = 0; e < 4; ++e) w[e] = tl[d * 33 + part * 4 + e];
    *(u32x4*)(vout + (long)d * Lpad + part * 8) = w;
  }
}

template <int HG>
__global__ __launch_bounds__(256) void qknorm_rope_rows_kernel(bf16_t* __restrict__ qkv, long ld, long bstride,
                                                               const bf16_t* __restrict__ q_scale, const bf16_t* __restrict__ k_scale,
                                                               const bf16_t* __restrict__ q_scale2, const bf16_t* __restrict__ k_scale2,
                                                               int split, const float* __restrict__ rope, long rope_bstride, int L,
                                                               int H, int parts) {
  const int tid = threadIdx.x;
  const int tok = blockIdx.x * 16 + (tid >> 4), sub = tid & 15, h0 = blockIdx.y * HG, b = blockIdx.z;
  if (tok >= L) return;
  const float* rp = rope + (long)b * rope_bstride + (long)tok * 128 + sub * 8;
  const f32x4 c0 = *(const f32x4*)rp;
  const f32x4 c1 = *(const f32x4*)(rp + 4);
  const float cs[8] = {c0[0], c0[1], c0[2], c0[3], c1[0], c1[1], c1[2], c1[3]};
  bf16_t* row = qkv + (long)b * bstride + (long)tok * ld + sub * 8;
#pragma unroll
  for (int which = 0; which < 2; ++which) {
    if (!(parts & (1 << which))) continue;
    const bf16_t* sc = (tok < split ? (which ? k_scale : q_scale) : (which ? k_scale2 : q_scale2)) + sub * 8;
    const u32x4 sw = *(const u32x4*)sc;
    float g[8];
#pragma unroll
    for (int e = 0; e < 4; ++e) { g[2 * e] = lo_bf(sw[e]); g[2 * e + 1] = hi_bf(sw[e]); }
    bf16_t* base = row + which * (H * 128) + h0 * 128;
    u32x4 w[HG];
#pragma unroll
    for (int hh = 0; hh < HG; ++hh) w[hh] = (h0 + hh < H) ? *(const u32x4*)(base + hh * 128) : u32x4{0u, 0u, 0u, 0u};
#pragma unroll
    for (int hh = 0; hh < HG; ++hh) {
      const u32x4 o = qknorm_rope8(w[hh], g, cs, (which == 0 && (parts & 8)) ? VC_QK_PRESCALE : 1.0f);
      if (h0 + hh < H) *(u32x4*)(base + hh * 128) = o;
    }
  }
}

}

int vc_ln_modulate2_launch(const VcLnStream* a, const VcLnStream* b, int64_t mod_bstride, int32_t D, const int32_t* step_ptr,
                           int64_t mod_step_stride, hipStream_t s, char* err, int errlen) {
  if (!a) { snprintf(err, errlen, "ln_modulate: null stream description"); return VC_ERR_ARG; }
  const VcLnStream* set[2] = {a, b};
  for (int i = 0; i < 2; ++i) {
    const VcLnStream* q = set[i];
    if (!q) continue;
    if (!q->x || !q->y || !q->shift || !q->scale) { snprintf(err, errlen, "ln_modulate: null pointer"); return VC_ERR_ARG; }
    if (q->rows <= 0 || D <= 0 || q->rows_per_batch <= 0) { snprintf(err, errlen, "ln_modulate: empty input rows=%d D=%d", q->rows, D); return VC_ERR_ARG; }
    if (D % 8 || D > 4096 || q->ldx % 8 || q->ldy % 8 || mod_bstride % 8 || mod_step_stride % 8) {
      snprintf(err, errlen, "ln_modulate: D=%d must be a multiple of 8 and <= 4096 with 16-B aligned strides", D); return VC_ERR_ARG; }
  }
  LnStream2 second = {nullptr, 0, nullptr, 0, nullptr, nullptr, 0, 1};
  if (b) second = LnStream2{(const bf16_t*)b->x, (long)b->ldx, (bf16_t*)b->y, (long)b->ldy, (const bf16_t*)b->shift,
                            (const bf16_t*)b->scale, b->rows, b->rows_per_batch};
  const dim3 grid((a->rows + second.rows + 3) / 4), block(256);
  if (D <= 3072)
    hipLaunchKernelGGL(ln_modulate_kernel<6>, grid, block, 0, s, (const bf16_t*)a->x, (long)a->ldx, (bf16_t*)a->y, (long)a->ldy,
                       (const bf16_t*)a->shift, (const bf16_t*)a->scale, (long)mod_bstride, a->rows, D, a->rows_per_batch,
                       step_ptr, (long)mod_step_stride, second);
  else
    hipLaunchKernelGGL(ln_modulate_kernel<8>, grid, block, 0, s, (const bf16_t*)a->x, (long)a->ldx, (bf16_t*)a->y, (long)a->ldy,
                       (const bf16_t*)a->shift, (const bf16_t*)a->scale, (long)mod_bstride, a->rows, D, a->rows_per_batch,
                       step_ptr, (long)mod_step_stride, second);
  hipError_t e = hipGetLastError();
  if (e != hipSuccess) { snprintf(err, errlen, "ln_modulate launch: %s", hipGetErrorString(e)); return VC_ERR_HIP; }
  return VC_OK;
}

int vc_ln_modulate_launch(const void* x, int64_t ldx, void* y, int64_t ldy, const void* shift, const void* scale,
                          int64_t mod_bstride, int32_t rows, int32_t D, int32_t rows_per_batch,
                          const int32_t* step_ptr, int64_t mod_step_stride, hipStream_t s, char* err, int errlen) {
  const VcLnStream a = {x, ldx, y, ldy, shift, scale, rows, rows_per_batch};
  return vc_ln_modulate2_launch(&a, nullptr, mod_bstride, D, step_ptr, mod_step_stride, s, err, errlen);
}

int vc_qknorm_rope_vt_launch(void* qkv, int64_t ld, int64_t bstride, const void* q_scale, const void* k_scale,
                             const void* q_scale2, const void* k_scale2, int32_t split, const float* rope, int64_t rope_bstride, void* vt, int32_t B, int32_t L, int32_t Lpad,
                             int32_t H, int32_t parts, hipStream_t s, char* err, int errlen) {
  if (!qkv || !q_scale || !k_scale || !rope || !vt) { snprintf(err, errlen, "qknorm_rope_vt: null pointer"); return VC_ERR_ARG; }
  if (parts <= 0 || parts > 15 || !(parts & 7) || ((parts & VC_QKN_QPRE) && !(parts & VC_QKN_Q))) {
    snprintf(err, errlen, "qknorm_rope_vt: parts=%d must be a non-empty subset of VC_QKN_Q | VC_QKN_K | VC_QKN_VT (+ VC_QKN_QPRE with VC_QKN_Q)", parts); return VC_ERR_ARG; }
  if (!q_scale2 || !k_scale2) { q_scale2 = q_scale; k_scale2 = k_scale; split = L; }
  if (B <= 0 || L <= 0 || H <= 0) { snprintf(err, errlen, "qknorm_rope_vt: empty problem"); return VC_ERR_ARG; }
  if (Lpad < L || Lpad % 64 || ld % 8 || bstride % 8) { snprintf(err, errlen, "qknorm_rope_vt: Lpad=%d must be a multiple of 64 >= L=%d; ld, bstride multiples of 8", Lpad, L); return VC_ERR_ARG; }
#ifndef VC_QKN_TILE_ONLY
  if (!(parts & VC_QKN_VT)) {
    constexpr int HG = 2;
    hipLaunchKernelGGL(qknorm_rope_rows_kernel<HG>, dim3((L + 15) / 16, (H + HG - 1) / HG, B), dim3(256), 0, s, (bf16_t*)qkv, (long)ld,
                       (long)bstride, (const bf16_t*)q_scale, (const bf16_t*)k_scale, (const bf16_t*)q_scale2, (const bf16_t*)k_scale2,
                       split, rope, (long)rope_bstride, L, H, parts);
    hipError_t e = hipGetLastError();
    if (e != hipSuccess) { snprintf(err, errlen, "qknorm_rope rows launch: %s", hipGetErrorString(e)); return VC_ERR_HIP; }
    return VC_OK;
  }
#endif
  const dim3 grid((L + 63) / 64, H, B), block(256);
  hipLaunchKernelGGL(qknorm_rope_vt_kernel, grid, block, 0, s, (bf16_t*)qkv, (long)ld, (long)bstride,
                     (const bf16_t*)q_scale, (const bf16_t*)k_scale, (const bf16_t*)q_scale2, (const bf16_t*)k_scale2, split,
                     rope, (long)rope_bstride, (bf16_t*)vt, L, Lpad, H, parts);
  hipError_t e = hipGetLastError();
  if (e != hipSuccess) { snprintf(err, errlen, "qknorm_rope_vt launch: %s", hipGetErrorString(e)); return VC_ERR_HIP; }
  return VC_OK;
}
```

visualcloze_amd/csrc/step_cache.hip:

```cpp
#include "common.h"
#include "vcloze_internal.h"

namespace {

constexpr int RC_THREADS = 256;
static_assert(RC_THREADS == VC_RESIDUAL_CHANGE_MAX_BLOCKS, "pass 2 holds one block partial per thread");

VC_DEV void block_tree_sum(float (&l0)[RC_THREADS], float (&l1)[RC_THREADS], float& s0, float& s1) {
  const int t = threadIdx.x;
  l0[t] = s0; l1[t] = s1;
  __syncthreads();
#pragma unroll
  for (int o = RC_THREADS / 2; o >= 1; o >>= 1) {
    if (t < o) { l0[t] += l0[t + o]; l1[t] += l1[t + o]; }
    __syncthreads();
  }
  s0 = l0[0]; s1 = l1[0];
  __syncthreads();
}

__global__ __launch_bounds__(RC_THREADS) void residual_change_kernel(const u32x4* __restrict__ h0, const u32x4* __restrict__ h1,
                                                                     const u32x4* __restrict__ p, u32x4* __restrict__ r,
                                                                     float* __restrict__ partial, long n8) {
  __shared__ float l0[RC_THREADS], l1[RC_THREADS];
  const int nblk = gridDim.x, b = blockIdx.y;
  const long base = (long)b * n8;
  float s0 = 0.0f, s1 = 0.0f;
  for (long c = (long)blockIdx.x * RC_THREADS + threadIdx.x; c < n8; c += (long)nblk * RC_THREADS) {
    const u32x4 a0 = h0[base + c], a1 = h1[base + c], pp = p[base + c];
    u32x4 o;
#pragma unroll
    for (int i = 0; i < 4; ++i) {
      const float rl = rbf(lo_bf(a1[i]) - lo_bf(a0[i])), rh = rbf(hi_bf(a1[i]) - hi_bf(a0[i]));
      const float pl = lo_bf(pp[i]), ph = hi_bf(pp[i]);
      s0 += fabsf(rl - pl); s1 += fabsf(pl);
      s0 += fabsf(rh - ph); s1 += fabsf(ph);
      o[i] = pack2bf(rl, rh);
    }
    r[base + c] = o;
  }
  block_tree_sum(l0, l1, s0, s1);
  if (threadIdx.x == 0) {
    partial[((long)b * nblk + blockIdx.x) * 2] = s0;
    partial[((long)b * nblk + blockIdx.x) * 2 + 1] = s1;
  }
}

__global__ __launch_bounds__(RC_THREADS) void residual_change_finish_kernel(const float* __restrict__ partial, float* __restrict__ sums,
                                                                            float* __restrict__ metric, int B, int nblk) {
  __shared__ float l0[RC_THREADS], l1[RC_THREADS];
  float m = 0.0f;
  for (int b = 0; b < B; ++b) {
    float s0 = 0.0f, s1 = 0.0f;
    if ((int)threadIdx.x < nblk) {
      s0 = partial[((long)b * nblk + threadIdx.x) * 2];
      s1 = partial[((long)b * nblk + threadIdx.x) * 2 + 1];
    }
    block_tree_sum(l0, l1, s0, s1);
    const float mb = s0 / s1;
    if (b == 0 || mb > m || mb != mb) m = (m != m) ? m : mb;
    if (threadIdx.x == 0 && sums) { sums[2 * b] = s0; sums[2 * b + 1] = s1; }
  }
  if (threadIdx.x == 0 && metric) *metric = m;
}

template <bool ADD>
__global__ __launch_bounds__(256) void residual_op_kernel(const u32x4* __restrict__ a, long a_bs, const u32x4* __restrict__ b, long b_bs,
                                                          u32x4* __restrict__ out, long o_bs, long n8) {
  const long c = (long)blockIdx.x * blockDim.x + threadIdx.x;
  if (c >= n8) return;
  const int s = blockIdx.y;
  const u32x4 x = a[s * a_bs + c], y = b[s * b_bs + c];
  u32x4 o;
#pragma unroll
  for (int i = 0; i < 4; ++i) {
    const float yl = ADD ? lo_bf(y[i]) : -lo_bf(y[i]), yh = ADD ? hi_bf(y[i]) : -hi_bf(y[i]);
    o[i] = pack2bf(lo_bf(x[i]) + yl, hi_bf(x[i]) + yh);
  }
  out[s * o_bs + c] = o;
}

inline bool aligned16(const void* p) { return ((uintptr_t)p & 15) == 0; }

}

#define VC_CHECK_LAUNCH(name)                                                                     \
  do {                                                                                            \
    hipError_t e_ = hipGetLastError();                                                            \
    if (e_ != hipSuccess) { snprintf(err, errlen, name " launch: %s", hipGetErrorString(e_)); return VC_ERR_HIP; } \
    return VC_OK;                                                                                 \
  } while (0)

int vc_residual_change_launch(const void* h0, const void* h1, const void* p, void* r, float* sums, float* metric, float* scratch,
                              int32_t B, int64_t n, hipStream_t s, char* err, int errlen) {
  if (!h0 || !h1 || !p || !r || !scratch || (!sums && !metric) || B <= 0 || B > 65535 || n <= 0) {
    snprintf(err, errlen, "residual_change: bad args");
    return VC_ERR_ARG;
  }
  if (n % 8 || !aligned16(h0) || !aligned16(h1) || !aligned16(p) || !aligned16(r)) {
    snprintf(err, errlen, "residual_change: n must be a multiple of 8 and every base 16-byte aligned");
    return VC_ERR_ARG;
  }
  const long n8 = n / 8;
  const long want = (n8 + RC_THREADS - 1) / RC_THREADS;
  const int nblk = (int)(want < VC_RESIDUAL_CHANGE_MAX_BLOCKS ? want : VC_RESIDUAL_CHANGE_MAX_BLOCKS);
  hipLaunchKernelGGL(residual_change_kernel, dim3(nblk, B), dim3(RC_THREADS), 0, s, (const u32x4*)h0, (const u32x4*)h1, (const u32x4*)p,
                     (u32x4*)r, scratch, n8);
  hipLaunchKernelGGL(residual_change_finish_kernel, dim3(1), dim3(RC_THREADS), 0, s, (const float*)scratch, sums, metric, (int)B, nblk);
  VC_CHECK_LAUNCH("residual_change");
}

int vc_residual_op_launch(int add, const void* a, int64_t a_bstride, const void* b, int64_t b_bstride, void* out, int64_t out_bstride,
                          int32_t B, int64_t n, hipStream_t s, char* err, int errlen) {
  const char* name = add ? "residual_add" : "residual_sub";
  if (!a || !b || !out || B <= 0 || B > 65535 || n <= 0 || a_bstride < 0 || b_bstride < 0 || out_bstride < (B > 1 ? n : 0)) {
    snprintf(err, errlen, "%s: bad args", name);
    return VC_ERR_ARG;
  }
  if (n % 8 || a_bstride % 8 || b_bstride % 8 || out_bstride % 8 || !aligned16(a) || !aligned16(b) || !aligned16(out)) {
    snprintf(err, errlen, "%s: n and the sample strides must be multiples of 8 and every base 16-byte aligned", name);
    return VC_ERR_ARG;
  }
  const long n8 = n / 8;
  const dim3 grid((unsigned)((n8 + 255) / 256), B), block(256);
  if (add) hipLaunchKernelGGL(residual_op_kernel<true>, grid, block, 0, s, (const u32x4*)a, (long)(a_bstride / 8), (const u32x4*)b,
                              (long)(b_bstride / 8), (u32x4*)out, (long)(out_bstride / 8), n8);
  else hipLaunchKernelGGL(residual_op_kernel<false>, grid, block, 0, s, (const u32x4*)a, (long)(a_bstride / 8), (const u32x4*)b,
                          (long)(b_bstride / 8), (u32x4*)out, (long)(out_bstride / 8), n8);
  hipError_t e_ = hipGetLastError();
  if (e_ != hipSuccess) { snprintf(err, errlen, "%s launch: %s", name, hipGetErrorString(e_)); return VC_ERR_HIP; }
  return VC_OK;
}
```

visualcloze_amd/csrc/vcloze_internal.h:

```cpp
#pragma once
#include <hip/hip_runtime.h>
#include <stdio.h>
#include "../../include/vcloze_hip.h"

constexpr int VC_MAX_DEVICES = 64;
inline int vc_device_index() {
  int d = 0;
  (void)hipGetDevice(&d);
  return d >= 0 && d < VC_MAX_DEVICES ? d : 0;
}
struct VcOncePerDevice {
  bool done[VC_MAX_DEVICES] = {};
  bool need() const { return !done[vc_device_index()]; }
  void mark() { done[vc_device_index()] = true; }
};
inline int vc_cu_count() {
  static int n[VC_MAX_DEVICES] = {};
  const int d = vc_device_index();
  if (n[d] == 0) {
    hipDeviceProp_t p;
    n[d] = hipGetDeviceProperties(&p, d) == hipSuccess && p.multiProcessorCount > 0 ? p.multiProcessorCount : 256;
  }
  return n[d];
}
int vc_gemm_launch(VcGemmArgs a, int tile_cfg, hipStream_t s, char* err, int errlen);
int vc_gemm_plan_impl(VcGemmArgs a, int tile_cfg, int32_t out[8], char* err, int errlen);
int vc_attention_launch(const VcAttention& a, hipStream_t s, char* err, int errlen);
int64_t vc_attention_scratch_bytes_impl();
int64_t vc_attention_flags_offset_impl();
int64_t vc_attention64_flags_bytes_impl(int n_cu);
int vc_attention64_launch(const VcAttention& a, bool tail_split, int n_cu, uint64_t* debug_ts, hipStream_t s, char* err, int errlen);
int64_t vc_attention64_scratch_bytes_impl(int n_cu);
int vc_ln_modulate2_launch(const VcLnStream* a, const VcLnStream* b, int64_t mod_bstride, int32_t D, const int32_t* step_ptr,
                           int64_t mod_step_stride, hipStream_t s, char* err, int errlen);
int vc_ln_modulate_launch(const void* x, int64_t ldx, void* y, int64_t ldy, const void* shift, const void* scale,
                          int64_t mod_bstride, int32_t rows, int32_t D, int32_t rows_per_batch,
                          const int32_t* step_ptr, int64_t mod_step_stride, hipStream_t s, char* err, int errlen);
int vc_qknorm_rope_vt_launch(void* qkv, int64_t ld, int64_t bstride, const void* q_scale, const void* k_scale,
                             const void* q_scale2, const void* k_scale2, int32_t split, const float* rope, int64_t rope_bstride, void* vt, int32_t B, int32_t L, int32_t Lpad,
                             int32_t H, int32_t parts, hipStream_t s, char* err, int errlen);
int vc_temb_launch(const float* t, const float* freqs, void* out, int n, int half, int round_t, hipStream_t s, char* err, int errlen);
int vc_silu_launch(const void* x, void* y, int64_t n, hipStream_t s, char* err, int errlen);
int vc_act2d_launch(const void* x, int64_t ldx, void* y, int64_t ldy, int32_t rows, int32_t cols, int32_t act, hipStream_t s,
                    char* err, int errlen);
int vc_gate_residual_launch(const void* y, int64_t ldy, const void* res, int64_t ldres, const void* gate, void* out, int64_t ldo,
                            int32_t rows, int32_t cols, const int32_t* step_ptr, int64_t gate_step_stride, hipStream_t s,
                            char* err, int errlen);
int vc_add3_launch(const void* a, const void* b, const void* c, void* y, int64_t n, int64_t bn, int64_t cn, hipStream_t s, char* err, int errlen);
int vc_concat_cols_launch(const void* x, int cx, const void* cond, int cc, void* out, int64_t rows, hipStream_t s, char* err, int errlen);
int vc_euler_launch(void* x, const void* v, const float* dts, const int32_t* step_ptr, int64_t n, hipStream_t s, char* err, int errlen);
int vc_euler_f32_launch(float* x32, void* shadow, const void* v, const float* dts, const int32_t* step_ptr, int64_t n, hipStream_t s,
                        char* err, int errlen);
inline int vc_evals_of(int method) {
  return method == VC_SOLVER_EULER ? 1 : method == VC_SOLVER_MIDPOINT ? 2 : method == VC_SOLVER_RK4 ? 4 : 0;
}
int vc_ode_stage_launch(int method, int stage, void* y, int state_is_bf16, const void* v, void* k, void* y_in, const float* dts,
                        const int32_t* eval_ptr, int64_t n, hipStream_t s, char* err, int errlen);
int vc_step_advance_launch(int32_t* step_ptr, hipStream_t s, char* err, int errlen);
int vc_residual_change_launch(const void* h0, const void* h1, const void* p, void* r, float* sums, float* metric, float* scratch,
                              int32_t B, int64_t n, hipStream_t s, char* err, int errlen);
int vc_residual_op_launch(int add, const void* a, int64_t a_bstride, const void* b, int64_t b_bstride, void* out, int64_t out_bstride,
                          int32_t B, int64_t n, hipStream_t s, char* err, int errlen);
int vc_pack_latent_launch(const void* in, void* out, int C, int h, int w, int64_t ld, int col0, hipStream_t s, char* err, int errlen);
int vc_pack_mask_launch(const void* in, void* out, int H, int W, int64_t ld, int col0, hipStream_t s, char* err, int errlen);
int vc_unpack_latent_launch(const void* in, int64_t ld, int col0, void* out, int C, int h, int w, hipStream_t s, char* err, int errlen);
int vc_sdedit_mix_launch(const void* noise, const void* latent, float strength, void* out, int64_t n, hipStream_t s, char* err, int errlen);
int vc_im2col3x3_launch(const void* src, void* dst, int H, int W, int C, int up, hipStream_t s, char* err, int errlen);
int vc_groupnorm_launch(const void* x, const void* gamma, const void* beta, void* y, void* scratch, int64_t scratch_bytes,
                        int64_t HW, int C, int G, float eps, int swish, hipStream_t s, char* err, int errlen);
int vc_softmax_rows_launch(void* x, int64_t ld, int rows, int cols, float scale, const void* bias, int64_t ldb, int causal_period,
                           hipStream_t s, char* err, int errlen);
int vc_transpose_launch(const void* src, int64_t lds_, void* dst, int64_t ldd, int R, int Cc, hipStream_t s, char* err, int errlen);
int vc_nchw_to_nhwc_launch(const void* src, int src_f32, void* dst, int C, int Cp, int64_t HW, float div, float add, hipStream_t s, char* err, int errlen);
int vc_nhwc_to_nchw_launch(const void* src, void* dst, int dst_f32, int C, int Cp, int64_t HW, hipStream_t s, char* err, int errlen);
int vc_gaussian_sample_launch(const void* moments, int Cp, const void* noise, void* out, int Z, int64_t HW, float scale, float shift,
                              hipStream_t s, char* err, int errlen);
int vc_embedding_launch(const int32_t* ids, const void* table, int64_t ldt, int V, void* out, int L, int D, hipStream_t s, char* err, int errlen);
int vc_rownorm_launch(const void* x, const void* w, const void* b, void* y, int rows, int D, float eps, int affine_ln, hipStream_t s, char* err, int errlen);
int vc_ewise_launch(const void* a, const void* b, void* y, int64_t n, int op, hipStream_t s, char* err, int errlen);
int vc_conv3x3_launch(const void* x, const void* w, const void* bias, void* out, int64_t ldc, const void* res, int64_t ldres,
                      const void* gate, int H, int W, int C, int O, int mode, hipStream_t s, char* err, int errlen);
int vc_lora_merge_launch(const void* w, int32_t w_is_f32, int64_t ldw, const void* lora_a, int64_t lda, const void* lora_b, int64_t ldb,
                         float scale, void* out, int64_t ldo, const void* bias, int32_t bias_is_f32, const void* lora_b_bias,
                         void* bias_out, int32_t out_features, int32_t in_features, int32_t rank, hipStream_t s, char* err, int errlen);

int vc_flux_create_impl(const VcFluxConfig* cfg, void** handle, char* err, int errlen);
int vc_flux_destroy_impl(void* handle, char* err, int errlen);
int vc_flux_bind_weight_impl(void* handle, const char* name, const void* w, const void* bias, int32_t rows, int32_t cols, int64_t ldw,
                             char* err, int errlen);
int64_t vc_flux_mod_offset_impl(void* handle, const char* name);
int vc_flux_set_option_impl(void* handle, const char* name, int32_t value, char* err, int errlen);
int64_t vc_flux_workspace_bytes_impl(void* handle, int32_t B, int32_t T, int32_t N, int32_t max_steps);
int vc_flux_prepare_impl(void* handle, const VcFluxInputs* in, void* workspace, int64_t workspace_bytes, hipStream_t s, char* err, int errlen);
int vc_flux_forward_impl(void* handle, const void* img, const float* timesteps, int32_t timesteps_is_bf16, void* out, hipStream_t s,
                         char* err, int errlen);
int vc_flux_sample_begin_impl(void* handle, int32_t method, const void* x, const void* cond, const float* t_grid, int32_t n_points, int32_t state_is_bf16,
                              hipStream_t s, char* err, int errlen);
int vc_flux_sample_steps_impl(void* handle, int32_t n_steps, void* trajectory, hipStream_t s, char* err, int errlen);
int vc_flux_profile_impl(void* handle, int32_t evaluations, VcFluxLaunchClass* out, int32_t capacity, int32_t* count, hipStream_t s,
                         char* err, int errlen);
int vc_flux_sample_end_impl(void* handle, void* x_out, hipStream_t s, char* err, int errlen);
int vc_flux_set_step_cache_impl(void* handle, float threshold, int32_t max_consecutive, char* err, int errlen);
int vc_flux_step_cache_stats_impl(void* handle, int32_t* computed, int32_t* reused, float* metrics, int32_t capacity, char* err, int errlen);
```

Baseline: 20.41 denoising-steps/sec.

## Alias text and image streams into the joint token buffer to drop concat copies

The text and image stream buffers now point into the combined sequence buffer X. Double-block GEMM epilogues and LayerNorm-modulate kernels take batch strides so they read and write there directly. This removes the per-evaluation copy of the text embeddings and the copy that concatenated both streams before the single blocks. The first double block reads the text-input projection straight from TXT0. The step-cache path now recomputes the image-input projection for its residual metric, adding a small GEMM there.

```diff
diff --git a/visualcloze_amd/csrc/api.hip b/visualcloze_amd/csrc/api.hip
--- a/visualcloze_amd/csrc/api.hip
+++ b/visualcloze_amd/csrc/api.hip
@@ -105,7 +105,7 @@
 int vc_step_advance(int32_t* step_ptr, void* stream) { return vc_step_advance_launch(step_ptr, S(stream), ERRBUF); }
 int vc_residual_change(const void* h0, const void* h1, const void* p, void* r, float* sums, float* metric, float* scratch, int32_t B,
                        int64_t n, void* stream) {
-  return vc_residual_change_launch(h0, h1, p, r, sums, metric, scratch, B, n, S(stream), ERRBUF);
+  return vc_residual_change_launch(h0, h1, n, p, r, sums, metric, scratch, B, n, S(stream), ERRBUF);
 }
 int vc_residual_sub(const void* a, int64_t a_bstride, const void* b, int64_t b_bstride, void* out, int64_t out_bstride, int32_t B,
                     int64_t n, void* stream) {
diff --git a/visualcloze_amd/csrc/flux_engine.hip b/visualcloze_amd/csrc/flux_engine.hip
--- a/visualcloze_amd/csrc/flux_engine.hip
+++ b/visualcloze_amd/csrc/flux_engine.hip
@@ -115,11 +115,11 @@
   const int64_t D = g.D, H = g.H, mlp = g.mlp, L = T + N, Lp = (L + 63) / 64 * 64;
   const int64_t in_ch = g.cfg.in_channels, out_ch = g.cfg.out_channels;
   Carver c{base};
-  f.XI = c.take<bf16_t>(B * N * D);          f.XT = c.take<bf16_t>(B * T * D);
   f.X = c.take<bf16_t>(B * L * D);           f.XH = c.take<bf16_t>(B * L * D);
+  f.XT = f.X;                                f.XI = f.X ? f.X + T * D : nullptr;
   f.QKV = c.take<bf16_t>(B * L * 3 * D);     f.VT = c.take<bf16_t>(B * H * 128 * Lp);
   f.CAT = c.take<bf16_t>(B * L * (D + mlp)); f.HID = c.take<bf16_t>(B * L * mlp);
-  f.TXT0 = c.take<bf16_t>(B * T * D);        f.XIN = c.take<bf16_t>(B * N * in_ch);
+  f.TXT0 = c.take<bf16_t>((B - 1) * L * D + T * D);   f.XIN = c.take<bf16_t>(B * N * in_ch);
   f.V = c.take<bf16_t>(B * N * out_ch);      f.XS = c.take<bf16_t>(B * N * out_ch);
   f.COND = c.take<bf16_t>(B * N * (in_ch - out_ch));
   f.MOD = c.take<bf16_t>((int64_t)S * B * g.n_mod);
@@ -310,17 +310,20 @@
 };
 inline const bf16_t* modp(Flux& f, int64_t off, int idx) { return f.MOD + off + (int64_t)idx * f.D; }
 
-int ln2(Flux& f, const Ctx& c, const DoubleW& w, int idx, Err e) {
-  VcLnStream a{f.XI, f.D, f.XH, f.D, modp(f, w.mod[0], idx), modp(f, w.mod[0], idx + 1), f.B * f.N, f.N};
-  VcLnStream b{f.XT, f.D, f.XH + (int64_t)f.B * f.N * f.D, f.D, modp(f, w.mod[1], idx), modp(f, w.mod[1], idx + 1), f.B * f.T, f.T};
+int ln2(Flux& f, const Ctx& c, const DoubleW& w, int idx, const bf16_t* txt, Err e) {
+  const int64_t xbs = (int64_t)f.L * f.D;
+  VcLnRows a{{f.XI, f.D, f.XH, f.D, modp(f, w.mod[0], idx), modp(f, w.mod[0], idx + 1), f.B * f.N, f.N}, xbs, 0};
+  VcLnRows b{{txt, f.D, f.XH + (int64_t)f.B * f.N * f.D, f.D, modp(f, w.mod[1], idx), modp(f, w.mod[1], idx + 1), f.B * f.T, f.T}, xbs, 0};
   TRY(prof_open(f, c.s, VC_LAUNCH_LN_MODULATE, 0, 0, 0, 0, 4.0 * f.B * f.L * f.D, e));
-  TRY(vc_ln_modulate2_launch(&a, &b, f.n_mod, f.D, c.step_ptr, c.mss, c.s, e.buf, e.len));
+  TRY(vc_ln_modulate_rows_launch(&a, &b, f.n_mod, f.D, c.step_ptr, c.mss, c.s, e.buf, e.len));
   return prof_close(f, c.s, e);
 }
-int ln1(Flux& f, const Ctx& c, int64_t mod, Err e) {
-  TRY(prof_open(f, c.s, VC_LAUNCH_LN_MODULATE, 0, 0, 0, 0, 4.0 * f.B * f.L * f.D, e));
-  TRY(vc_ln_modulate_launch(f.X, f.D, f.XH, f.D, modp(f, mod, 0), modp(f, mod, 1), f.n_mod, f.B * f.L, f.D, f.L, c.step_ptr, c.mss,
-                            c.s, e.buf, e.len));
+int ln1(Flux& f, const Ctx& c, int64_t mod, int row0, Err e) {
+  const int rows = f.L - row0;
+  const int64_t bs = (int64_t)f.L * f.D, off = (int64_t)row0 * f.D;
+  VcLnRows a{{f.X + off, f.D, f.XH + off, f.D, modp(f, mod, 0), modp(f, mod, 1), f.B * rows, rows}, bs, bs};
+  TRY(prof_open(f, c.s, VC_LAUNCH_LN_MODULATE, 0, 0, 0, 0, 4.0 * f.B * rows * f.D, e));
+  TRY(vc_ln_modulate_rows_launch(&a, nullptr, f.n_mod, f.D, c.step_ptr, c.mss, c.s, e.buf, e.len));
   return prof_close(f, c.s, e);
 }
 
@@ -356,14 +359,15 @@
   return prof_close(f, c.s, e);
 }
 
-int double_block(Flux& f, const Ctx& c, const DoubleW& w, Err e) {
+int double_block(Flux& f, const Ctx& c, const DoubleW& w, bool first, Err e) {
   const int B = f.B, T = f.T, N = f.N, L = f.L, D = f.D, mlp = f.mlp;
   const int64_t ldq = 3 * D, ldc = D + mlp;
   bf16_t* XH_I = f.XH; bf16_t* XH_T = f.XH + (int64_t)B * N * D;
   bf16_t* HID_I = f.HID; bf16_t* HID_T = f.HID + (int64_t)B * N * mlp;
   bf16_t* streams[2] = {f.XI, f.XT};
   const int rows[2] = {N, T};
-  TRY(ln2(f, c, w, 0, e));
+  const int64_t xbs = (int64_t)L * D;
+  TRY(ln2(f, c, w, 0, first ? f.TXT0 : f.XT, e));
   {
     VcGemmProblem p[2] = {prob(XH_I, D, w.qkv[0], f.QKV + (int64_t)T * ldq, ldq, B * N), prob(XH_T, D, w.qkv[1], f.QKV, ldq, B * T)};
     p[0].c_rpb = N; p[1].c_rpb = T;
@@ -377,10 +381,12 @@
     for (int k = 0; k < 2; ++k) {
       p[k].res = streams[k]; p[k].ldres = D; p[k].gate = modp(f, w.mod[k], 2); p[k].gate_bstride = f.n_mod;
       p[k].rows_per_batch = rows[k]; p[k].a_rpb = rows[k]; p[k].a_bstride = (int64_t)L * ldc;
-    }
+      p[k].c_rpb = rows[k]; p[k].c_bstride = xbs;
+    }
+    if (first) p[1].res = f.TXT0;
     TRY(gemm(f, p, 2, VC_EPI_GATE_RES, c.step_ptr, c.mss, c.s, e));
   }
-  TRY(ln2(f, c, w, 3, e));
+  TRY(ln2(f, c, w, 3, f.XT, e));
   {
     VcGemmProblem p[2] = {prob(XH_I, D, w.mlp0[0], HID_I, mlp, B * N), prob(XH_T, D, w.mlp0[1], HID_T, mlp, B * T)};
     TRY(gemm(f, p, 2, VC_EPI_GELU, nullptr, 0, c.s, e));
@@ -389,6 +395,7 @@
     VcGemmProblem p[2] = {prob(HID_I, mlp, w.mlp2[0], f.XI, D, B * N), prob(HID_T, mlp, w.mlp2[1], f.XT, D, B * T)};
     for (int k = 0; k < 2; ++k) {
       p[k].res = streams[k]; p[k].ldres = D; p[k].gate = modp(f, w.mod[k], 5); p[k].gate_bstride = f.n_mod; p[k].rows_per_batch = rows[k];
+      p[k].c_rpb = rows[k]; p[k].c_bstride = xbs;
     }
     TRY(gemm(f, p, 2, VC_EPI_GATE_RES, c.step_ptr, c.mss, c.s, e));
   }
@@ -398,7 +405,7 @@
 int single_block(Flux& f, const Ctx& c, const SingleW& w, Err e) {
   const int M = f.B * f.L, D = f.D, mlp = f.mlp;
   const int64_t ldc = D + mlp;
-  TRY(ln1(f, c, w.mod, e));
+  TRY(ln1(f, c, w.mod, 0, e));
   {
     VcGemmProblem p = prob(f.XH, D, w.qkv, f.QKV, 3 * D, M);
     with_vt(f, p, f.L, 0, w.qs, w.ks);
@@ -416,22 +423,23 @@
   HIP(hipMemcpyAsync(dst, src, (size_t)bytes, hipMemcpyDeviceToDevice, s), "hipMemcpyAsync");
   return VC_OK;
 }
+int d2d_rows(bf16_t* dst, int64_t dst_bs, const bf16_t* src, int64_t src_bs, int B, int64_t n, hipStream_t s, Err e) {
+  if (dst_bs == n && src_bs == n) return d2d(dst, src, B * n * 2, s, e);
+  for (int b = 0; b < B; ++b) TRY(d2d(dst + b * dst_bs, src + b * src_bs, n * 2, s, e));
+  return VC_OK;
+}
 
 int eval_inputs(Flux& f, bool concat, const void* img_rows, hipStream_t s, Err e) {
   const int B = f.B, T = f.T, N = f.N, D = f.D;
   const int in_ch = f.cfg.in_channels, out_ch = f.cfg.out_channels;
   if (concat) TRY(vc_concat_cols_launch(f.method == VC_SOLVER_EULER ? f.XS : f.YIN, out_ch, f.COND, in_ch - out_ch, f.XIN, (int64_t)B * N, s, e.buf, e.len));
-  TRY(d2d(f.XT, f.TXT0, (int64_t)B * T * D * 2, s, e));
-  return lin(f, f.img_in, img_rows ? img_rows : f.XIN, in_ch, f.XI, D, B * N, VC_EPI_BIAS, s, e);
+  if (f.dbl.empty()) TRY(d2d_rows(f.XT, (int64_t)f.L * D, f.TXT0, (int64_t)f.L * D, B, (int64_t)T * D, s, e));
+  VcGemmProblem p = prob(img_rows ? img_rows : f.XIN, in_ch, f.img_in, f.XI, D, B * N);
+  p.c_rpb = N; p.c_bstride = (int64_t)f.L * D;
+  return gemm(f, &p, 1, VC_EPI_BIAS, nullptr, 0, s, e);
 }
 int eval_blocks(Flux& f, const Ctx& c, size_t first, Err e) {
-  const int B = f.B, T = f.T, N = f.N, L = f.L, D = f.D;
-  hipStream_t s = c.s;
-  for (size_t i = first; i < f.dbl.size(); ++i) TRY(double_block(f, c, f.dbl[i], e));
-  for (int b = 0; b < B; ++b) {
-    TRY(d2d(f.X + (int64_t)b * L * D, f.XT + (int64_t)b * T * D, (int64_t)T * D * 2, s, e));
-    TRY(d2d(f.X + ((int64_t)b * L + T) * D, f.XI + (int64_t)b * N * D, (int64_t)N * D * 2, s, e));
-  }
+  for (size_t i = first; i < f.dbl.size(); ++i) TRY(double_block(f, c, f.dbl[i], i == 0, e));
   for (auto& w : f.sgl) TRY(single_block(f, c, w, e));
   return VC_OK;
 }
@@ -440,7 +448,7 @@
   const int out_ch = f.cfg.out_channels;
   const int32_t* step_ptr = c.step_ptr;
   hipStream_t s = c.s;
-  TRY(ln1(f, c, f.final_mod, e));
+  TRY(ln1(f, c, f.final_mod, T, e));
   VcGemmProblem p = prob(f.XH + (int64_t)T * D, D, f.final_lin, out ? out : f.V, out_ch, B * N);
   p.a_rpb = N; p.a_bstride = (int64_t)L * D;
   TRY(gemm(f, &p, 1, VC_EPI_BIAS, nullptr, 0, s, e));
@@ -466,9 +474,9 @@
   const int64_t nd = (int64_t)f.N * f.D;
   Ctx c{f.STEP, s, (int64_t)f.B * f.n_mod};
   TRY(eval_inputs(f, true, nullptr, s, e));
-  TRY(d2d(f.X, f.XI, f.B * nd * 2, s, e));
-  TRY(double_block(f, c, f.dbl[0], e));
-  TRY(vc_residual_change_launch(f.X, f.XI, f.SC_P, f.SC_RS, nullptr, f.SC_METRIC, f.SC_PART, f.B, nd, s, e.buf, e.len));
+  TRY(double_block(f, c, f.dbl[0], true, e));
+  TRY(lin(f, f.img_in, f.XIN, f.cfg.in_channels, f.HID, f.D, f.B * f.N, VC_EPI_BIAS, s, e));
+  TRY(vc_residual_change_launch(f.HID, f.XI, (int64_t)f.L * f.D, f.SC_P, f.SC_RS, nullptr, f.SC_METRIC, f.SC_PART, f.B, nd, s, e.buf, e.len));
   HIP(hipMemcpyAsync(f.sc_host, f.SC_METRIC, sizeof(float), hipMemcpyDeviceToHost, s), "hipMemcpyAsync(D2H)");
   return VC_OK;
 }
@@ -476,7 +484,7 @@
   const int64_t nd = (int64_t)f.N * f.D;
   Ctx c{f.STEP, s, (int64_t)f.B * f.n_mod};
   TRY(d2d(f.SC_P, f.SC_RS, f.B * nd * 2, s, e));
-  TRY(d2d(f.SC_RS, f.XI, f.B * nd * 2, s, e));
+  TRY(d2d_rows(f.SC_RS, nd, f.XI, (int64_t)f.L * f.D, f.B, nd, s, e));
   TRY(eval_blocks(f, c, 1, e));
   TRY(vc_residual_op_launch(0, f.X + (int64_t)f.T * f.D, (int64_t)f.L * f.D, f.SC_RS, nd, f.SC_R, nd, f.B, nd, s, e.buf, e.len));
   return eval_output(f, c, nullptr, euler, e);
@@ -484,7 +492,7 @@
 int cache_tail_reuse(Flux& f, bool euler, hipStream_t s, Err e) {
   const int64_t nd = (int64_t)f.N * f.D;
   Ctx c{f.STEP, s, (int64_t)f.B * f.n_mod};
-  TRY(vc_residual_op_launch(1, f.XI, nd, f.SC_R, nd, f.X + (int64_t)f.T * f.D, (int64_t)f.L * f.D, f.B, nd, s, e.buf, e.len));
+  TRY(vc_residual_op_launch(1, f.XI, (int64_t)f.L * f.D, f.SC_R, nd, f.XI, (int64_t)f.L * f.D, f.B, nd, s, e.buf, e.len));
   return eval_output(f, c, nullptr, euler, e);
 }
 
@@ -783,7 +791,11 @@
   TRY(stage_end(f, s, e));
   HIP(hipMemsetAsync(f.VT, 0, (size_t)B * f.H * 128 * f.Lp * 2, s), "hipMemsetAsync");
   HIP(hipMemsetAsync((char*)f.ATT_SCRATCH + vc_attention_flags_offset_impl(), 0, (size_t)vc_attention64_flags_bytes_impl(f.n_cu), s), "hipMemsetAsync");
-  TRY(lin(f, f.txt_in, in->txt, f.cfg.context_in_dim, f.TXT0, D, B * T, VC_EPI_BIAS, s, e));
+  {
+    VcGemmProblem p = prob(in->txt, f.cfg.context_in_dim, f.txt_in, f.TXT0, D, B * T);
+    p.c_rpb = T; p.c_bstride = (int64_t)L * D;
+    TRY(gemm(f, &p, 1, VC_EPI_BIAS, nullptr, 0, s, e));
+  }
   if (f.cfg.guidance_embed) {
     TRY(vc_temb_launch(f.G32, f.FREQS, f.GE, B, 128, in->guidance_is_bf16, s, e.buf, e.len));
     TRY(lin(f, f.guidance_in[0], f.GE, 256, f.GH, D, B, VC_EPI_SILU, s, e));
diff --git a/visualcloze_amd/csrc/norm.hip b/visualcloze_amd/csrc/norm.hip
--- a/visualcloze_amd/csrc/norm.hip
+++ b/visualcloze_amd/csrc/norm.hip
@@ -4,7 +4,7 @@
 namespace {
 
 struct LnStream2 {
-  const bf16_t* x; long ldx; bf16_t* y; long ldy; const bf16_t* shift; const bf16_t* scale; int rows; int rows_per_batch;
+  const bf16_t* x; long ldx; bf16_t* y; long ldy; const bf16_t* shift; const bf16_t* scale; int rows; int rows_per_batch; long xbs, ybs;
 };
 
 template <int NCH>
@@ -12,18 +12,20 @@
                                                           long ldy, const bf16_t* __restrict__ shift,
                                                           const bf16_t* __restrict__ scale, long mod_bstride, int rows,
                                                           int D, int rows_per_batch, const int* __restrict__ step_ptr,
-                                                          long mod_step_stride, const LnStream2 second) {
+                                                          long mod_step_stride, long xbs, long ybs, const LnStream2 second) {
   const int lane = threadIdx.x & 63;
   int row = blockIdx.x * 4 + (threadIdx.x >> 6);
   if (row >= rows) {
     row -= rows;
     if (row >= second.rows) return;
     x = second.x; ldx = second.ldx; y = second.y; ldy = second.ldy; shift = second.shift; scale = second.scale;
-    rows_per_batch = second.rows_per_batch;
-  }
-  long moff = (long)(row / rows_per_batch) * mod_bstride;
+    rows_per_batch = second.rows_per_batch; xbs = second.xbs; ybs = second.ybs;
+  }
+  const int batch = row / rows_per_batch;
+  row -= batch * rows_per_batch;
+  long moff = (long)batch * mod_bstride;
   if (step_ptr) moff += (long)(*step_ptr) * mod_step_stride;
-  const bf16_t* xr = x + (long)row * ldx;
+  const bf16_t* xr = x + (long)batch * xbs + (long)row * ldx;
   float v[NCH][8];
   float sum = 0.f;
 #pragma unroll
@@ -51,7 +53,7 @@
     }
   }
   const float rstd = 1.0f / sqrtf(wave_sum(ss) / (float)D + 1e-6f);
-  bf16_t* yr = y + (long)row * ldy;
+  bf16_t* yr = y + (long)batch * ybs + (long)row * ldy;
 #pragma unroll
   for (int c = 0; c < NCH; ++c) {
     const int idx = c * 512 + lane * 8;
@@ -171,33 +173,40 @@
 
 }
 
+int vc_ln_modulate_rows_launch(const VcLnRows* a, const VcLnRows* b, int64_t mod_bstride, int32_t D, const int32_t* step_ptr,
+                               int64_t mod_step_stride, hipStream_t s, char* err, int errlen) {
+  if (!a) { snprintf(err, errlen, "ln_modulate: null stream description"); return VC_ERR_ARG; }
+  const VcLnRows* set[2] = {a, b};
+  LnStream2 k[2] = {{nullptr, 0, nullptr, 0, nullptr, nullptr, 0, 1, 0, 0}, {nullptr, 0, nullptr, 0, nullptr, nullptr, 0, 1, 0, 0}};
+  for (int i = 0; i < 2; ++i) {
+    if (!set[i]) continue;
+    const VcLnStream* q = &set[i]->s;
+    if (!q->x || !q->y || !q->shift || !q->scale) { snprintf(err, errlen, "ln_modulate: null pointer"); return VC_ERR_ARG; }
+    if (q->rows <= 0 || D <= 0 || q->rows_per_batch <= 0) { snprintf(err, errlen, "ln_modulate: empty input rows=%d D=%d", q->rows, D); return VC_ERR_ARG; }
+    if (D % 8 || D > 4096 || q->ldx % 8 || q->ldy % 8 || mod_bstride % 8 || mod_step_stride % 8 || set[i]->x_bstride % 8 || set[i]->y_bstride % 8 ||
+        set[i]->x_bstride < 0 || set[i]->y_bstride < 0) {
+      snprintf(err, errlen, "ln_modulate: D=%d must be a multiple of 8 and <= 4096 with 16-B aligned strides", D); return VC_ERR_ARG; }
+    k[i] = LnStream2{(const bf16_t*)q->x, (long)q->ldx, (bf16_t*)q->y, (long)q->ldy, (const bf16_t*)q->shift, (const bf16_t*)q->scale, q->rows,
+                     q->rows_per_batch, (long)(set[i]->x_bstride ? set[i]->x_bstride : q->rows_per_batch * q->ldx),
+                     (long)(set[i]->y_bstride ? set[i]->y_bstride : q->rows_per_batch * q->ldy)};
+  }
+  const dim3 grid((k[0].rows + k[1].rows + 3) / 4), block(256);
+  if (D <= 3072)
+    hipLaunchKernelGGL(ln_modulate_kernel<6>, grid, block, 0, s, k[0].x, k[0].ldx, k[0].y, k[0].ldy, k[0].shift, k[0].scale, (long)mod_bstride,
+                       k[0].rows, D, k[0].rows_per_batch, step_ptr, (long)mod_step_stride, k[0].xbs, k[0].ybs, k[1]);
+  else
+    hipLaunchKernelGGL(ln_modulate_kernel<8>, grid, block, 0, s, k[0].x, k[0].ldx, k[0].y, k[0].ldy, k[0].shift, k[0].scale, (long)mod_bstride,
+                       k[0].rows, D, k[0].rows_per_batch, step_ptr, (long)mod_step_stride, k[0].xbs, k[0].ybs, k[1]);
+  hipError_t e = hipGetLastError();
+  if (e != hipSuccess) { snprintf(err, errlen, "ln_modulate launch: %s", hipGetErrorString(e)); return VC_ERR_HIP; }
+  return VC_OK;
+}
+
 int vc_ln_modulate2_launch(const VcLnStream* a, const VcLnStream* b, int64_t mod_bstride, int32_t D, const int32_t* step_ptr,
                            int64_t mod_step_stride, hipStream_t s, char* err, int errlen) {
   if (!a) { snprintf(err, errlen, "ln_modulate: null stream description"); return VC_ERR_ARG; }
-  const VcLnStream* set[2] = {a, b};
-  for (int i = 0; i < 2; ++i) {
-    const VcLnStream* q = set[i];
-    if (!q) continue;
-    if (!q->x || !q->y || !q->shift || !q->scale) { snprintf(err, errlen, "ln_modulate: null pointer"); return VC_ERR_ARG; }
-    if (q->rows <= 0 || D <= 0 || q->rows_per_batch <= 0) { snprintf(err, errlen, "ln_modulate: empty input rows=%d D=%d", q->rows, D); return VC_ERR_ARG; }
-    if (D % 8 || D > 4096 || q->ldx % 8 || q->ldy % 8 || mod_bstride % 8 || mod_step_stride % 8) {
-      snprintf(err, errlen, "ln_modulate: D=%d must be a multiple of 8 and <= 4096 with 16-B aligned strides", D); return VC_ERR_ARG; }
-  }
-  LnStream2 second = {nullptr, 0, nullptr, 0, nullptr, nullptr, 0, 1};
-  if (b) second = LnStream2{(const bf16_t*)b->x, (long)b->ldx, (bf16_t*)b->y, (long)b->ldy, (const bf16_t*)b->shift,
-                            (const bf16_t*)b->scale, b->rows, b->rows_per_batch};
-  const dim3 grid((a->rows + second.rows + 3) / 4), block(256);
-  if (D <= 3072)
-    hipLaunchKernelGGL(ln_modulate_kernel<6>, grid, block, 0, s, (const bf16_t*)a->x, (long)a->ldx, (bf16_t*)a->y, (long)a->ldy,
-                       (const bf16_t*)a->shift, (const bf16_t*)a->scale, (long)mod_bstride, a->rows, D, a->rows_per_batch,
-                       step_ptr, (long)mod_step_stride, second);
-  else
-    hipLaunchKernelGGL(ln_modulate_kernel<8>, grid, block, 0, s, (const bf16_t*)a->x, (long)a->ldx, (bf16_t*)a->y, (long)a->ldy,
-                       (const bf16_t*)a->shift, (const bf16_t*)a->scale, (long)mod_bstride, a->rows, D, a->rows_per_batch,
-                       step_ptr, (long)mod_step_stride, second);
-  hipError_t e = hipGetLastError();
-  if (e != hipSuccess) { snprintf(err, errlen, "ln_modulate launch: %s", hipGetErrorString(e)); return VC_ERR_HIP; }
-  return VC_OK;
+  const VcLnRows ra = {*a, 0, 0}, rb = {b ? *b : *a, 0, 0};
+  return vc_ln_modulate_rows_launch(&ra, b ? &rb : nullptr, mod_bstride, D, step_ptr, mod_step_stride, s, err, errlen);
 }
 
 int vc_ln_modulate_launch(const void* x, int64_t ldx, void* y, int64_t ldy, const void* shift, const void* scale,
diff --git a/visualcloze_amd/csrc/step_cache.hip b/visualcloze_amd/csrc/step_cache.hip
--- a/visualcloze_amd/csrc/step_cache.hip
+++ b/visualcloze_amd/csrc/step_cache.hip
@@ -21,13 +21,13 @@
 
 __global__ __launch_bounds__(RC_THREADS) void residual_change_kernel(const u32x4* __restrict__ h0, const u32x4* __restrict__ h1,
                                                                      const u32x4* __restrict__ p, u32x4* __restrict__ r,
-                                                                     float* __restrict__ partial, long n8) {
+                                                                     float* __restrict__ partial, long n8, long h1_bs) {
   __shared__ float l0[RC_THREADS], l1[RC_THREADS];
   const int nblk = gridDim.x, b = blockIdx.y;
   const long base = (long)b * n8;
   float s0 = 0.0f, s1 = 0.0f;
   for (long c = (long)blockIdx.x * RC_THREADS + threadIdx.x; c < n8; c += (long)nblk * RC_THREADS) {
-    const u32x4 a0 = h0[base + c], a1 = h1[base + c], pp = p[base + c];
+    const u32x4 a0 = h0[base + c], a1 = h1[(long)b * h1_bs + c], pp = p[base + c];
     u32x4 o;
 #pragma unroll
     for (int i = 0; i < 4; ++i) {
@@ -65,8 +65,8 @@
 }
 
 template <bool ADD>
-__global__ __launch_bounds__(256) void residual_op_kernel(const u32x4* __restrict__ a, long a_bs, const u32x4* __restrict__ b, long b_bs,
-                                                          u32x4* __restrict__ out, long o_bs, long n8) {
+__global__ __launch_bounds__(256) void residual_op_kernel(const u32x4* a, long a_bs, const u32x4* __restrict__ b, long b_bs,
+                                                          u32x4* out, long o_bs, long n8) {
   const long c = (long)blockIdx.x * blockDim.x + threadIdx.x;
   if (c >= n8) return;
   const int s = blockIdx.y;
@@ -91,13 +91,13 @@
     return VC_OK;                                                                                 \
   } while (0)
 
-int vc_residual_change_launch(const void* h0, const void* h1, const void* p, void* r, float* sums, float* metric, float* scratch,
-                              int32_t B, int64_t n, hipStream_t s, char* err, int errlen) {
-  if (!h0 || !h1 || !p || !r || !scratch || (!sums && !metric) || B <= 0 || B > 65535 || n <= 0) {
+int vc_residual_change_launch(const void* h0, const void* h1, int64_t h1_bstride, const void* p, void* r, float* sums, float* metric,
+                              float* scratch, int32_t B, int64_t n, hipStream_t s, char* err, int errlen) {
+  if (!h0 || !h1 || !p || !r || !scratch || (!sums && !metric) || B <= 0 || B > 65535 || n <= 0 || h1_bstride < n) {
     snprintf(err, errlen, "residual_change: bad args");
     return VC_ERR_ARG;
   }
-  if (n % 8 || !aligned16(h0) || !aligned16(h1) || !aligned16(p) || !aligned16(r)) {
+  if (n % 8 || h1_bstride % 8 || !aligned16(h0) || !aligned16(h1) || !aligned16(p) || !aligned16(r)) {
     snprintf(err, errlen, "residual_change: n must be a multiple of 8 and every base 16-byte aligned");
     return VC_ERR_ARG;
   }
@@ -105,7 +105,7 @@
   const long want = (n8 + RC_THREADS - 1) / RC_THREADS;
   const int nblk = (int)(want < VC_RESIDUAL_CHANGE_MAX_BLOCKS ? want : VC_RESIDUAL_CHANGE_MAX_BLOCKS);
   hipLaunchKernelGGL(residual_change_kernel, dim3(nblk, B), dim3(RC_THREADS), 0, s, (const u32x4*)h0, (const u32x4*)h1, (const u32x4*)p,
-                     (u32x4*)r, scratch, n8);
+                     (u32x4*)r, scratch, n8, (long)(h1_bstride / 8));
   hipLaunchKernelGGL(residual_change_finish_kernel, dim3(1), dim3(RC_THREADS), 0, s, (const float*)scratch, sums, metric, (int)B, nblk);
   VC_CHECK_LAUNCH("residual_change");
 }
diff --git a/visualcloze_amd/csrc/vcloze_internal.h b/visualcloze_amd/csrc/vcloze_internal.h
--- a/visualcloze_amd/csrc/vcloze_internal.h
+++ b/visualcloze_amd/csrc/vcloze_internal.h
@@ -31,6 +31,9 @@
 int64_t vc_attention64_flags_bytes_impl(int n_cu);
 int vc_attention64_launch(const VcAttention& a, bool tail_split, int n_cu, uint64_t* debug_ts, hipStream_t s, char* err, int errlen);
 int64_t vc_attention64_scratch_bytes_impl(int n_cu);
+struct VcLnRows { VcLnStream s; int64_t x_bstride, y_bstride; };
+int vc_ln_modulate_rows_launch(const VcLnRows* a, const VcLnRows* b, int64_t mod_bstride, int32_t D, const int32_t* step_ptr,
+                               int64_t mod_step_stride, hipStream_t s, char* err, int errlen);
 int vc_ln_modulate2_launch(const VcLnStream* a, const VcLnStream* b, int64_t mod_bstride, int32_t D, const int32_t* step_ptr,
                            int64_t mod_step_stride, hipStream_t s, char* err, int errlen);
 int vc_ln_modulate_launch(const void* x, int64_t ldx, void* y, int64_t ldy, const void* shift, const void* scale,
@@ -57,8 +60,8 @@
 int vc_ode_stage_launch(int method, int stage, void* y, int state_is_bf16, const void* v, void* k, void* y_in, const float* dts,
                         const int32_t* eval_ptr, int64_t n, hipStream_t s, char* err, int errlen);
 int vc_step_advance_launch(int32_t* step_ptr, hipStream_t s, char* err, int errlen);
-int vc_residual_change_launch(const void* h0, const void* h1, const void* p, void* r, float* sums, float* metric, float* scratch,
-                              int32_t B, int64_t n, hipStream_t s, char* err, int errlen);
+int vc_residual_change_launch(const void* h0, const void* h1, int64_t h1_bstride, const void* p, void* r, float* sums, float* metric,
+                              float* scratch, int32_t B, int64_t n, hipStream_t s, char* err, int errlen);
 int vc_residual_op_launch(int add, const void* a, int64_t a_bstride, const void* b, int64_t b_bstride, void* out, int64_t out_bstride,
                           int32_t B, int64_t n, hipStream_t s, char* err, int errlen);
 int vc_pack_latent_launch(const void* in, void* out, int C, int h, int w, int64_t ld, int col0, hipStream_t s, char* err, int errlen);
```

Result: no change. 20.33 denoising-steps/sec (-0.4%).
